# JiapengWu/TeMP

Hardware: AMD Instinct MI355X
Metric: edges/sec (fwd+bwd) RGCN+GRU seq_len=15 (higher is better)
Workload: dtype f32

## Files before the change

### include/temp_amd.h

```cpp
#ifndef TEMP_AMD_H
#define TEMP_AMD_H

#include <stddef.h>
#include <stdint.h>

#ifdef __cplusplus
extern "C" {
#endif

#define TEMP_ABI_VERSION 2

enum {
  TEMP_OK = 0,
  TEMP_E_BADARG = 1,
  TEMP_E_UNSUPPORTED = 2,
  TEMP_E_WORKSPACE = 3,
  TEMP_E_LAUNCH = 4
};

enum { TEMP_ACT_NONE = 0, TEMP_ACT_RELU = 1 };
enum { TEMP_GRU_TORCH = 0,
       TEMP_GRU_TYPE1 = 1 };

int temp_abi_version(void);
// ... 183 lines not shown
size_t temp_gru_bwd_workspace(int n, int d, int variant);
int temp_gru_bwd(int n, int d, int variant,
                 const float* x, const float* prev, const int32_t* prev_idx , const float* dt,
                 float lambda, const float* decay_wb ,
                 const float* w_ih, const float* w_hh,
                 const float* saved, const float* d_h_out,
                 float* d_x, float* d_prev, float* d_w_ih, float* d_w_hh, float* d_b_ih, float* d_b_hh,
                 float* d_decay_wb ,
                 void* workspace, size_t workspace_bytes, void* stream);

int temp_decay_rows(int n, int d, const float* x, const float* dt, float lambda, float* out, void* stream);

int temp_gru_input_gates(int n, int d, int variant, const float* x, const float* w_ih, const float* b_ih, float* gi, void* stream);
int temp_gru_input_gates_multi(int count, const int* ns, int d, int variant, const float* const* xs, const float* const* w_ihs,
                               const float* const* b_ihs, float* const* gis, void* stream);
int temp_gru_input_gates_gather_multi(int count, const int* ns, int d, int variant, const float* const* xs, const int32_t* const* x_idx,
                                      const float* const* w_ihs, const float* const* b_ihs, float* const* gis, void* stream);
int temp_gru_cell_fwd(int n, int d, int variant, const float* gi, const float* prev, const int32_t* prev_idx ,
                      const float* dt, float lambda, const float* w_hh, const float* b_hh,
                      float* h_out, float* saved, size_t saved_plane, void* stream);
int temp_gru_cell_bwd(int n, int d, int variant, const float* saved, size_t saved_plane,
                      const float* dh_up , const float* d_prev_next , const int32_t* next_idx ,
                      const float* dt, float lambda, const float* w_hh,
                      float* dgi, float* dgh, float* decv, float* d_prev, void* stream);
typedef struct TempGruCellFwd {
  int32_t n; const float* gi; const float* prev ;
  const int32_t* prev_idx ; const float* dt;
  const float* w_hh; const float* b_hh; float* h_out; float* saved ;
} TempGruCellFwd;
typedef struct TempGruCellBwd {
  int32_t n; const float* saved; const float* dh_up ; const float* d_prev_next ;
  const int32_t* next_idx ; const float* dt; const float* w_hh;
  float* dgi; float* dgh; float* decv; float* d_prev;
  int32_t no_prev;
} TempGruCellBwd;
int temp_gru_cell_fwd_multi(int count, const TempGruCellFwd* cells, int d, int variant, float lambda, size_t saved_plane, void* stream);
int temp_gru_cell_bwd_multi(int count, const TempGruCellBwd* cells, int d, int variant, float lambda, size_t saved_plane, void* stream);
size_t temp_gru_weight_grads_workspace(int n, int d, int variant);
int temp_gru_weight_grads(int n, int d, int variant, const float* x, const float* hdec, const float* dgi, const float* dgh,
                          const float* w_ih, float* d_x , float* d_w_ih, float* d_w_hh, float* d_b_ih, float* d_b_hh,
                          void* workspace, size_t workspace_bytes, void* stream);
size_t temp_gru_weight_grads_multi_workspace(int count, const int* ns, int d, int variant);
int temp_gru_weight_grads_multi(int count, const int* ns, int d, int variant, const float* const* xs, const float* const* hdecs,
                                const float* const* dgis, const float* const* dghs, const float* const* w_ihs, float* const* d_xs,
                                float* d_w, float* d_b, void* workspace, size_t workspace_bytes, void* stream);

size_t temp_gru_grads_g4_workspace(int count, const int* ns, int d);
int temp_gru_grads_g4(int count, const int* ns, int d, const float* const* xs, const float* const* hdecs, const float* const* g4s,
                      const float* const* w_ihs, float* const* d_xs, float* d_w, float* d_b, void* workspace, size_t workspace_bytes,
                      void* stream);
int temp_gru_grads_g4_keys(int count, const int* ns, int d, const float* const* xs, const float* const* hdecs, const float* const* g4s,
                           const float* const* w_ihs, float* const* d_xs, float* d_w, float* d_b, const uint32_t* const* g4_row_keys,
                           const uint32_t* const* g4_col_keys, const uint32_t* const* x_col_keys ,
                           void* workspace, size_t workspace_bytes, void* stream);
int temp_gru_grads_g4_rows_supported(int count, const int* ns, int d, int table_rows);
int temp_gru_grads_g4_rows(int count, const int* ns, int d, const float* table, int table_rows, const int32_t* const* x_rows,
                           const float* const* hdecs, const float* const* g4s, const float* const* w_ihs, float* const* d_xs, float* d_w,
                           float* d_b, const uint32_t* const* g4_row_keys, const uint32_t* const* g4_col_keys,
                           const uint32_t* const* x_col_keys, void* workspace, size_t workspace_bytes, void* stream);

#define TEMP_CHAIN_HAS_PREV (1 << 30)
#define TEMP_CHAIN_TRACKS 32
#define TEMP_CHAIN_MAX_RNN 4
#define TEMP_CHAIN_MAX_UP 8
typedef struct TempChainDecay { const float* wb[TEMP_CHAIN_MAX_RNN]; } TempChainDecay;
typedef struct TempChainOffset { const float* table; const int32_t* index; int32_t n_rows; } TempChainOffset;
typedef struct TempGruChain {
  int32_t d, variant, n_panels, n_steps;
  int32_t max_steps;
  const int32_t* panel; const int32_t* rows; const int32_t* sinfo;
  const float* dt;
  float lambda;
  size_t saved_plane;
  int32_t n_rnn;
  const float* packed[TEMP_CHAIN_MAX_RNN];
  const float* b_hh[TEMP_CHAIN_MAX_RNN];
  const int32_t* gi_index;
  int32_t pack_layout;
  const TempChainDecay* decay;
  const TempChainOffset* offset;
} TempGruChain;
enum { TEMP_CHAIN_PACK_F32 = 1, TEMP_CHAIN_PACK_BX = 2, TEMP_CHAIN_PACK_HX = 3, TEMP_CHAIN_PACK_HX_X = 4 };
int temp_gru_chain_pack_layout(int d);
int temp_gru_chain_supported(int d);
size_t temp_gru_chain_pack_floats(int d);
int temp_gru_chain_pack(int d, const float* w_hh, float* packed, void* stream);
int temp_gru_chain_pack_multi(int count, int d, const float* const* w_hh, float* const* packed, void* stream);
int temp_gru_chain_pack_multi_layout(int layout, int count, int d, const float* const* w_hh, float* const* packed, void* stream);
size_t temp_gru_chain_pack_x_floats(int d);
int temp_gru_chain_pack_x_multi(int count, int d, const float* const* w_hh, const float* const* w_ih, float* const* packed, void* stream);
typedef struct TempChainFwd {
  const float* gi; const float* x; const int32_t* x_index; const float* const* b_ih;
  float* h_out; float* saved;
} TempChainFwd;
int temp_gru_chain_fwd(const TempGruChain* c, const TempChainFwd* io, void* stream);
typedef struct TempChainBwd {
  const float* saved; int32_t n_up; const float* const* up;
  float* dgi; float* dgh; float* g4; uint32_t* row_keys; uint32_t* col_keys;
  float* d_arg; float* d_state;
} TempChainBwd;
int temp_gru_chain_bwd(const TempGruChain* c, const TempChainBwd* io, void* stream);
int temp_gru_chain_fwd_x_supported(int d, int variant, int max_steps);
long long temp_gru_chain_fwd_x_launches(void);
int temp_gru_chain_keys_supported(int d);
int temp_gru_chain_decay_supported(int d, int variant);
long long temp_gru_chain_decay_launches(void);
int temp_gru_chain_offset_supported(int d, int variant);
int temp_gru_chain_offset_layout(int d);
long long temp_gru_chain_offset_launches(void);
size_t temp_gru_chain_decay_reduce_workspace(const TempGruChain* c);
int temp_gru_chain_decay_reduce(const TempGruChain* c, const float* d_arg, float* d_wb, void* ws, size_t ws_bytes, void* stream);

int temp_gather_rows(int n, int d, const float* table, const int32_t* idx, float* out, void* stream);
size_t temp_keys_cols_size(int d);
int temp_absmax_keys(int n, int d, const float* x, int ldx, uint32_t* row_keys, uint32_t* col_keys, void* stream);
int temp_gather_rows_keys(int n, int d, const float* table, const int32_t* idx, float* out, uint32_t* row_keys, uint32_t* col_keys, void* stream);
int temp_linear_keys(int M, int N, int K, const float* A, int lda, const uint32_t* a_keys, const float* B, int ldb, int trans_b, float* C, int ldc,
                     void* stream);
int temp_gru_input_gates_gather_multi_keys(int count, const int* ns, int d, int variant, const float* const* xs, const int32_t* const* x_idx,
                                           const uint32_t* const* x_keys, const float* const* w_ihs, const float* const* b_ihs, float* const* gis,
                                           void* stream);
int temp_scatter_add_rows(int n, int d, const float* src, const int32_t* idx, float* table, void* stream);
size_t temp_segment_sum_rows_workspace(int n_seg, int n_rows, int d);
int temp_segment_sum_rows(int n_seg, int n_rows, int d, const int32_t* seg_ptr, const int32_t* order, const float* src, float* out,
                          void* workspace, size_t workspace_bytes, void* stream);
int temp_segment_sum_rows_relu(int n_seg, int n_rows, int d, const int32_t* seg_ptr, const int32_t* order, const float* src, const float* relu_of,
                               float* out, void* workspace, size_t workspace_bytes, void* stream);

int temp_diachronic_rows_fwd(int B, int N, int d, const float* ent, const float* w, const float* b, const float* t, float* out, void* stream);
int temp_diachronic_rows_bwd(int B, int N, int d, const float* ent, const float* w, const float* b, const float* t, const float* d_out, float* d_ent,
                             float* d_w, float* d_b, void* stream);

#define TEMP_HYPERPLANE_TILE_ROWS 32
#define TEMP_HYPERPLANE_CHUNK 8
size_t temp_hyperplane_rows_bwd_workspace(int B, int N, int d);
int temp_hyperplane_rows_fwd(int B, int N, int d, const float* table, const float* w, float* out, void* stream);
int temp_hyperplane_rows_bwd(int B, int N, int d, const float* table, const float* w, const float* d_out, float* d_table, float* d_w,
                             void* workspace, size_t workspace_bytes, void* stream);

int temp_linear(int M, int N, int K, const float* A, int lda, const float* B, int ldb, int trans_b, float* C, int ldc, void* stream);
int temp_linear_t(int M, int N, int K, const float* A, int lda, const float* B, int ldb, int trans_b, float* Ct, int ldct, void* stream);
typedef struct TempLinearProblem { int M; const float* A; const float* B; float* C; } TempLinearProblem;
int temp_linear_multi(int count, const TempLinearProblem* probs, int N, int K, int lda, int ldb, int trans_b, int ldc, void* stream);
// ... 124 lines not shown
```

### temp_amd/_lib.py

```python
import ctypes
import threading
import os

_HERE = os.path.dirname(os.path.abspath(__file__))
LIB_PATH = os.path.join(_HERE, "libtemp_amd.so")

c_i32p = ctypes.POINTER(ctypes.c_int32)
c_f32p = ctypes.POINTER(ctypes.c_float)
c_vp = ctypes.c_void_p

ACT_NONE, ACT_RELU = 0, 1
GRU_TORCH, GRU_TYPE1 = 0, 1
CHUNK = 64
CHUNK_REL = 128


class TempEdgeView(ctypes.Structure):
    _fields_ = [("n_seg", ctypes.c_int32), ("n_edges", ctypes.c_int32), ("a", c_vp), ("b", c_vp),
                ("n_chunks", ctypes.c_int32), ("chunk_seg", c_vp), ("chunk_beg", c_vp), ("chunk_end", c_vp),
                ("chunk_slot", c_vp), ("n_partial", ctypes.c_int32), ("n_fix", ctypes.c_int32),
                ("fix_seg", c_vp), ("fix_slot", c_vp), ("fix_cnt", c_vp)]


class TempMembers(ctypes.Structure):
    _fields_ = [("n_members", ctypes.c_int32), ("max_nodes", ctypes.c_int32), ("max_edges", ctypes.c_int32),
                ("max_chunks", ctypes.c_int32 * 3), ("node_off", c_vp), ("edge_off", c_vp), ("chunk_off", c_vp), ("fix_off", c_vp)]


class TempGraph(ctypes.Structure):
    _fields_ = [("n_nodes", ctypes.c_int32), ("n_edges", ctypes.c_int32), ("nnorm", c_vp), ("in_deg", c_vp),
                ("out_deg", c_vp), ("by_dst", TempEdgeView), ("by_src", TempEdgeView), ("by_rel", TempEdgeView),
                ("members", TempMembers)]


class TempPairView(ctypes.Structure):
    _fields_ = [("n_table", ctypes.c_int32), ("n_rel_rows", ctypes.c_int32), ("fwd_row", c_vp), ("by_pair", TempEdgeView)]


ABI_VERSION = 2
OPT_MFMA_BF16X3, OPT_TN_SPLIT, OPT_RGCN_SCALAR, OPT_GEMM_STREAM, OPT_GRU_STREAM, OPT_RGCN_TILE, OPT_DEBUG, OPT_OVERLAP, OPT_GEMM_RESIDENT, OPT_MFMA_F16X2, OPT_RGCN_PAIR = range(11)


class TempGruCellFwd(ctypes.Structure):
    _fields_ = [("n", ctypes.c_int32), ("gi", c_vp), ("prev", c_vp), ("prev_idx", c_vp), ("dt", c_vp), ("w_hh", c_vp),
                ("b_hh", c_vp), ("h_out", c_vp), ("saved", c_vp)]


class TempGruCellBwd(ctypes.Structure):
    _fields_ = [("n", ctypes.c_int32), ("saved", c_vp), ("dh_up", c_vp), ("d_prev_next", c_vp), ("next_idx", c_vp), ("dt", c_vp),
                ("w_hh", c_vp), ("dgi", c_vp), ("dgh", c_vp), ("decv", c_vp), ("d_prev", c_vp), ("no_prev", ctypes.c_int32)]


CHAIN_HAS_PREV = 1 << 30
CHAIN_TRACKS = 32
CHAIN_MAX_RNN = 4
CHAIN_MAX_UP = 8
CHAIN_MAX_STEPS = 64
CHAIN_PACK_F32, CHAIN_PACK_BX, CHAIN_PACK_HX, CHAIN_PACK_HX_X = 1, 2, 3, 4


class TempChainDecay(ctypes.Structure):
    _fields_ = [("wb", c_vp * CHAIN_MAX_RNN)]


class TempChainOffset(ctypes.Structure):
    _fields_ = [("table", c_vp), ("index", c_vp), ("n_rows", ctypes.c_int32)]


class TempGruChain(ctypes.Structure):
    _fields_ = [("d", ctypes.c_int32), ("variant", ctypes.c_int32), ("n_panels", ctypes.c_int32), ("n_steps", ctypes.c_int32),
                ("max_steps", ctypes.c_int32), ("panel", c_vp), ("rows", c_vp), ("sinfo", c_vp), ("dt", c_vp), ("lambda_", ctypes.c_float),
                ("saved_plane", ctypes.c_size_t), ("n_rnn", ctypes.c_int32), ("packed", c_vp * CHAIN_MAX_RNN), ("b_hh", c_vp * CHAIN_MAX_RNN),
                ("gi_index", c_vp), ("pack_layout", ctypes.c_int32),
                ("decay", ctypes.POINTER(TempChainDecay)), ("offset", ctypes.POINTER(TempChainOffset))]


class TempChainFwd(ctypes.Structure):
    _fields_ = [(n, c_vp) for n in ("gi", "x", "x_index", "b_ih", "h_out", "saved")]


class TempChainBwd(ctypes.Structure):
    _fields_ = [("saved", c_vp), ("n_up", ctypes.c_int32), ("up", c_vp)] + [(n, c_vp) for n in ("dgi", "dgh", "g4", "row_keys", "col_keys", "d_arg", "d_state")]


class TempSubsampleJob(ctypes.Structure):
    _fields_ = [("n_nodes", ctypes.c_int32), ("n_edges", ctypes.c_int32), ("keep", ctypes.c_int32), ("seed", ctypes.c_uint64),
                ("parent", c_vp), ("child", c_vp), ("eid", c_vp),
                ("off_a", ctypes.c_int32 * 3), ("off_b", ctypes.c_int32 * 3), ("off_chunk_beg", ctypes.c_int32 * 3),
                ("off_chunk_end", ctypes.c_int32 * 3), ("off_chunk_seg", ctypes.c_int32 * 3), ("n_chunks", ctypes.c_int32 * 3),
                ("off_in_deg", ctypes.c_int32), ("off_out_deg", ctypes.c_int32), ("off_nnorm", ctypes.c_int32),
                ("keep_mask", c_vp), ("scratch", c_vp)]


class TempDropout(ctypes.Structure):
    _fields_ = [("p", ctypes.c_float), ("seed", ctypes.c_uint64)]


class TempAttn(ctypes.Structure):
    _fields_ = [("n", ctypes.c_int32), ("D", ctypes.c_int32), ("heads", ctypes.c_int32), ("T", ctypes.c_int32),
                ("q", c_vp), ("ldq", ctypes.c_int32), ("kh", c_vp), ("vh", c_vp), ("ldh", ctypes.c_int32),
                ("kc", c_vp), ("vc", c_vp), ("ldc", ctypes.c_int32), ("idx", c_vp), ("decay", c_vp)]


class TempAttnSplit(ctypes.Structure):
    _fields_ = [("pa", c_vp), ("ia", c_vp), ("lda", ctypes.c_int32), ("pb", c_vp), ("ib", c_vp), ("ldb", ctypes.c_int32)]


class TempLinearProblem(ctypes.Structure):
    _fields_ = [("M", ctypes.c_int32), ("A", c_vp), ("B", c_vp), ("C", c_vp)]


# ... 18 lines not shown
    "temp_get_option": (_I, [_I]),
    "temp_scratch_refused": (ctypes.c_longlong, []),
    "temp_f16_launches": (ctypes.c_longlong, []),
    "temp_gemm_route_launches": (ctypes.c_longlong, [_I, _I]),
    "temp_rgcn_route_launches": (ctypes.c_longlong, [_I, _I]),
    "temp_tile_launches": (ctypes.c_longlong, []),
    "temp_set_debug_buffer": (None, [c_vp, _SZ]),
    "temp_rgcn_fwd_workspace": (_SZ, [_G, _I]),
    "temp_rgcn_fwd": (_I, [_G, c_vp, c_vp, _I, _I, _I, _I, c_vp, c_vp, c_vp, _I, c_vp, c_vp, _SZ, c_vp, c_vp]),
    "temp_rgcn_bwd_workspace": (_SZ, [_G, _I, _I, _I, _I]),
    "temp_rgcn_bwd": (_I, [_G, c_vp, c_vp, c_vp, _I, _I, _I, _I, c_vp, c_vp, _I, _I, c_vp, c_vp, c_vp, c_vp, c_vp, _SZ, c_vp, c_vp]),
    "temp_rgcn_bwd_dh": (_I, [_G, c_vp, c_vp, _I, _I, _I, _I, c_vp, c_vp, _I, c_vp, c_vp, c_vp, c_vp, _SZ, c_vp, c_vp]),
    "temp_rgcn_bwd_weights": (_I, [_G, c_vp, c_vp, c_vp, _I, _I, _I, _I, _I, c_vp, c_vp, c_vp, c_vp, _SZ, c_vp]),
    "temp_rgcn_table_fwd_workspace": (_SZ, [_G, _I, _I]),
    "temp_rgcn_table_fwd": (_I, [_G, c_vp, c_vp, _I, _I, _I, _I, _I, c_vp, c_vp, c_vp, _I, c_vp, c_vp, _SZ, c_vp, c_vp]),
    "temp_rgcn_table_bwd_workspace": (_SZ, [_G, _I, _I, _I, _I]),
    "temp_rgcn_table_bwd": (_I, [_G, c_vp, c_vp, c_vp, c_vp, _I, c_vp, c_vp, _I, _I, _I, _I, c_vp, c_vp, _I, _I, c_vp, c_vp, c_vp, c_vp,
                                 c_vp, _SZ, c_vp, c_vp]),
    "temp_pair_launches": (ctypes.c_longlong, []),
    "temp_expand_chunk_segments": (_I, [_I, c_vp, c_vp, c_vp, _I, c_vp, c_vp]),
    "temp_rgcn_pair_supported": (_I, [_I, _I, _I]),
    "temp_rgcn_pair_fwd_workspace": (_SZ, [_G, _PV, _I]),
    "temp_rgcn_pair_fwd": (_I, [_G, _PV, c_vp, c_vp, _I, _I, _I, _I, _I, c_vp, c_vp, c_vp, _I, c_vp, c_vp, _SZ, c_vp, c_vp]),
    "temp_rgcn_pair_bwd_workspace": (_SZ, [_G, _PV, _I, _I, _I]),
    "temp_rgcn_pair_bwd": (_I, [_G, _PV, c_vp, c_vp, c_vp, c_vp, _I, c_vp, c_vp, _I, _I, _I, _I, c_vp, c_vp, _I, _I, c_vp, c_vp, c_vp, c_vp,
                                c_vp, _SZ, c_vp, c_vp]),
    "temp_rgcn_isolated_fwd": (_I, [_I, _I, c_vp, c_vp, c_vp, _I, c_vp, c_vp, c_vp]),
    "temp_rgcn_isolated_bwd_workspace": (_SZ, [_I, _I]),
    "temp_rgcn_isolated_bwd": (_I, [_I, _I, c_vp, c_vp, c_vp, c_vp, _I, _I, c_vp, c_vp, c_vp, c_vp, _SZ, c_vp, c_vp]),
    "temp_gru_fwd": (_I, [_I, _I, _I, c_vp, c_vp, c_vp, c_vp, _F, c_vp, c_vp, c_vp, c_vp, c_vp, c_vp, c_vp, c_vp]),
    "temp_gru_bwd_workspace": (_SZ, [_I, _I, _I]),
    "temp_gru_bwd": (_I, [_I, _I, _I, c_vp, c_vp, c_vp, c_vp, _F, c_vp, c_vp, c_vp, c_vp, c_vp,
                          c_vp, c_vp, c_vp, c_vp, c_vp, c_vp, c_vp, c_vp, _SZ, c_vp]),
    "temp_decay_rows": (_I, [_I, _I, c_vp, c_vp, _F, c_vp, c_vp]),
    "temp_gru_input_gates": (_I, [_I, _I, _I, c_vp, c_vp, c_vp, c_vp, c_vp]),
    "temp_gru_input_gates_multi": (_I, [_I, c_vp, _I, _I, c_vp, c_vp, c_vp, c_vp, c_vp]),
    "temp_gru_input_gates_gather_multi": (_I, [_I, c_vp, _I, _I, c_vp, c_vp, c_vp, c_vp, c_vp, c_vp]),
    "temp_gru_cell_fwd": (_I, [_I, _I, _I, c_vp, c_vp, c_vp, c_vp, _F, c_vp, c_vp, c_vp, c_vp, _SZ, c_vp]),
    "temp_gru_cell_bwd": (_I, [_I, _I, _I, c_vp, _SZ, c_vp, c_vp, c_vp, c_vp, _F, c_vp, c_vp, c_vp, c_vp, c_vp, c_vp]),
    "temp_gru_cell_fwd_multi": (_I, [_I, ctypes.POINTER(TempGruCellFwd), _I, _I, _F, _SZ, c_vp]),
    "temp_gru_cell_bwd_multi": (_I, [_I, ctypes.POINTER(TempGruCellBwd), _I, _I, _F, _SZ, c_vp]),
    "temp_gru_weight_grads_workspace": (_SZ, [_I, _I, _I]),
    "temp_gru_weight_grads": (_I, [_I, _I, _I, c_vp, c_vp, c_vp, c_vp, c_vp, c_vp, c_vp, c_vp, c_vp, c_vp, c_vp, _SZ, c_vp]),
    "temp_gru_weight_grads_multi_workspace": (ctypes.c_size_t, [_I, c_vp, _I, _I]),
    "temp_gru_weight_grads_multi": (_I, [_I, c_vp, _I, _I, c_vp, c_vp, c_vp, c_vp, c_vp, c_vp, c_vp, c_vp, c_vp, ctypes.c_size_t, c_vp]),
    "temp_gru_chain_supported": (_I, [_I]),
    "temp_gru_chain_pack_floats": (_SZ, [_I]),
    "temp_gru_chain_pack": (_I, [_I, c_vp, c_vp, c_vp]),
    "temp_gru_chain_pack_multi": (_I, [_I, _I, ctypes.POINTER(c_vp), ctypes.POINTER(c_vp), c_vp]),
    "temp_gru_chain_fwd": (_I, [ctypes.POINTER(TempGruChain), ctypes.POINTER(TempChainFwd), c_vp]),
    "temp_gru_chain_pack_layout": (_I, [_I]),
    "temp_gru_chain_fwd_x_supported": (_I, [_I, _I, _I]),
    "temp_gru_chain_pack_x_floats": (_SZ, [_I]),
    "temp_gru_chain_pack_x_multi": (_I, [_I, _I, ctypes.POINTER(c_vp), ctypes.POINTER(c_vp), ctypes.POINTER(c_vp), c_vp]),
    "temp_gru_chain_fwd_x_launches": (ctypes.c_longlong, []),
    "temp_gru_chain_bwd": (_I, [ctypes.POINTER(TempGruChain), ctypes.POINTER(TempChainBwd), c_vp]),
    "temp_gru_chain_keys_supported": (_I, [_I]),
    "temp_gru_chain_decay_supported": (_I, [_I, _I]),
    "temp_gru_chain_decay_reduce_workspace": (_SZ, [ctypes.POINTER(TempGruChain)]),
    "temp_gru_chain_decay_reduce": (_I, [ctypes.POINTER(TempGruChain), c_vp, c_vp, c_vp, _SZ, c_vp]),
    "temp_gru_chain_decay_launches": (ctypes.c_longlong, []),
    "temp_gru_chain_offset_supported": (_I, [_I, _I]),
    "temp_gru_chain_offset_layout": (_I, [_I]),
    "temp_gru_chain_pack_multi_layout": (_I, [_I, _I, _I, ctypes.POINTER(c_vp), ctypes.POINTER(c_vp), c_vp]),
    "temp_gru_chain_offset_launches": (ctypes.c_longlong, []),
    "temp_gru_grads_g4_keys": (_I, [_I, c_vp, _I, c_vp, c_vp, c_vp, c_vp, c_vp, c_vp, c_vp, c_vp, c_vp, c_vp, c_vp, ctypes.c_size_t, c_vp]),
    "temp_gru_grads_g4_rows_supported": (_I, [_I, c_vp, _I, _I]),
    "temp_gru_grads_g4_rows": (_I, [_I, c_vp, _I, c_vp, _I, c_vp, c_vp, c_vp, c_vp, c_vp, c_vp, c_vp, c_vp, c_vp, c_vp, c_vp, ctypes.c_size_t, c_vp]),
    "temp_gru_grads_g4_workspace": (ctypes.c_size_t, [_I, c_vp, _I]),
    "temp_gru_grads_g4": (_I, [_I, c_vp, _I, c_vp, c_vp, c_vp, c_vp, c_vp, c_vp, c_vp, c_vp, ctypes.c_size_t, c_vp]),
    "temp_gather_rows": (_I, [_I, _I, c_vp, c_vp, c_vp, c_vp]),
    "temp_keys_cols_size": (_SZ, [_I]),
    "temp_absmax_keys": (_I, [_I, _I, c_vp, _I, c_vp, c_vp, c_vp]),
    "temp_gather_rows_keys": (_I, [_I, _I, c_vp, c_vp, c_vp, c_vp, c_vp, c_vp]),
    "temp_linear_keys": (_I, [_I, _I, _I, c_vp, _I, c_vp, c_vp, _I, _I, c_vp, _I, c_vp]),
    "temp_gru_input_gates_gather_multi_keys": (_I, [_I, c_vp, _I, _I, c_vp, c_vp, c_vp, c_vp, c_vp, c_vp, c_vp]),
    "temp_scatter_add_rows": (_I, [_I, _I, c_vp, c_vp, c_vp, c_vp]),
    "temp_segment_sum_rows_workspace": (_SZ, [_I, _I, _I]),
    "temp_segment_sum_rows": (_I, [_I, _I, _I, c_vp, c_vp, c_vp, c_vp, c_vp, _SZ, c_vp]),
    "temp_segment_sum_rows_relu": (_I, [_I, _I, _I, c_vp, c_vp, c_vp, c_vp, c_vp, c_vp, _SZ, c_vp]),
    "temp_diachronic_rows_fwd": (_I, [_I, _I, _I, c_vp, c_vp, c_vp, c_vp, c_vp, c_vp]),
    "temp_diachronic_rows_bwd": (_I, [_I, _I, _I, c_vp, c_vp, c_vp, c_vp, c_vp, c_vp, c_vp, c_vp, c_vp]),
    "temp_hyperplane_rows_bwd_workspace": (_SZ, [_I, _I, _I]),
    "temp_hyperplane_rows_fwd": (_I, [_I, _I, _I, c_vp, c_vp, c_vp, c_vp]),
    "temp_hyperplane_rows_bwd": (_I, [_I, _I, _I, c_vp, c_vp, c_vp, c_vp, c_vp, c_vp, _SZ, c_vp]),
    "temp_linear": (_I, [_I, _I, _I, c_vp, _I, c_vp, _I, _I, c_vp, _I, c_vp]),
    "temp_linear_t": (_I, [_I, _I, _I, c_vp, _I, c_vp, _I, _I, c_vp, _I, c_vp]),
    "temp_linear_multi": (_I, [_I, ctypes.POINTER(TempLinearProblem), _I, _I, _I, _I, _I, _I, c_vp]),
    "temp_linear_tn_workspace": (_SZ, [_I, _I, _I]),
    "temp_linear_tn_multi_workspace": (_SZ, [_I, _I, _I, _I]),
    "temp_linear_tn_multi": (_I, [_I, ctypes.POINTER(TempLinearProblem), _I, _I, _I, _I, _I, c_vp, _SZ, c_vp]),
    "temp_linear_tn": (_I, [_I, _I, _I, c_vp, _I, c_vp, _I, c_vp, _I, c_vp, _SZ, c_vp]),
    "temp_gather_ce_fwd": (_I, [_I, _I, _I, c_vp, c_vp, c_vp, c_vp, c_vp]),
    "temp_gather_ce_bwd": (_I, [_I, _I, _I, c_vp, c_vp, c_vp, c_vp, _F, c_vp, c_vp, c_vp]),
    "temp_bilinear_query_fwd": (_I, [_I, _I, _I, c_vp, c_vp, c_vp, c_vp, c_vp, c_vp, c_vp]),
    "temp_bilinear_query_bwd": (_I, [_I, _I, _I, c_vp, c_vp, c_vp, c_vp, c_vp, c_vp, c_vp, c_vp, c_vp]),
    "temp_l1_ce_fwd": (_I, [_I, _I, _I, c_vp, c_vp, c_vp, c_vp, c_vp, c_vp, c_vp, c_vp]),
    "temp_l1_ce_bwd_q": (_I, [_I, _I, _I, c_vp, c_vp, c_vp, c_vp, c_vp, c_vp, c_vp, _F, c_vp, c_vp, c_vp, c_vp]),
    "temp_l1_ce_bwd_table": (_I, [_I, _I, _I, c_vp, c_vp, c_vp, c_vp, c_vp, c_vp, c_vp]),
    "temp_l1_scores": (_I, [_I, _I, _I, c_vp, c_vp, _I, c_vp, c_vp]),
    "temp_gated_query_fwd": (_I, [_I, _I, _I, c_vp, c_vp, c_vp, c_vp, c_vp, c_vp, c_vp, c_vp, c_vp, c_vp]),
    "temp_gated_query_bwd": (_I, [_I, _I, _I, c_vp, c_vp, c_vp, c_vp, c_vp, c_vp, c_vp, c_vp, c_vp, c_vp, c_vp, c_vp, c_vp, c_vp]),
    "temp_gather_ce_mix_fwd": (_I, [_I, _I, _I, c_vp, c_vp, c_vp, c_vp, c_vp, c_vp, c_vp]),
    "temp_gather_ce_mix_bwd": (_I, [_I, _I, _I, c_vp, c_vp, c_vp, c_vp, c_vp, c_vp, _F, c_vp, c_vp, c_vp, c_vp, c_vp]),
    "temp_l1_mix_ce_fwd": (_I, [_I, _I, _I, c_vp, c_vp, c_vp, c_vp, c_vp, c_vp, c_vp, c_vp, c_vp, c_vp]),
    "temp_l1_mix_ce_bwd_q": (_I, [_I, _I, _I, c_vp, c_vp, c_vp, c_vp, c_vp, c_vp, c_vp, c_vp, c_vp, _F, c_vp, c_vp, c_vp, c_vp, c_vp]),
    "temp_l1_mix_ce_bwd_table": (_I, [_I, _I, _I, c_vp, c_vp, c_vp, c_vp, c_vp, c_vp, c_vp, c_vp, c_vp, c_vp]),
    "temp_l1_mix_scores": (_I, [_I, _I, _I, c_vp, c_vp, c_vp, c_vp, _I, c_vp, c_vp]),
    "temp_assemble_views": (_I, [_I, c_vp, c_vp, c_vp, c_vp, c_vp, c_vp]),
    "temp_subsample_views": (_I, [_I, ctypes.POINTER(TempSubsampleJob), c_vp]),
    "temp_corrupt_sample": (_I, [_I, _I, _I, ctypes.c_uint64, c_vp, c_vp, c_vp, c_vp, c_vp, c_vp]),
    "temp_filtered_rank": (_I, [_I, _I, _I, c_vp, c_vp, c_vp, c_vp, c_vp, c_vp]),
    "temp_filtered_topk": (_I, [_I, _I, _I, _I, _I, c_vp, c_vp, c_vp, c_vp, _I, c_vp, c_vp, c_vp]),
    "temp_filtered_topk_mix": (_I, [_I, _I, _I, _I, _I, c_vp, c_vp, c_vp, c_vp, c_vp, c_vp, _I, c_vp, c_vp, c_vp]),
    "temp_grad_norm_workspace": (_SZ, [_I]),
    "temp_grad_norm_clip": (_I, [_I, _I, c_vp, ctypes.c_double, c_vp, _SZ, c_vp, c_vp]),
    "temp_adam_clip_step": (_I, [_I, _I, c_vp, c_vp, c_vp]),
    "temp_sa_attn_fwd": (_I, [ctypes.POINTER(TempAttn), c_vp, c_vp, c_vp, c_vp]),
    "temp_sa_attn_bwd": (_I, [ctypes.POINTER(TempAttn), c_vp, c_vp, c_vp, c_vp, c_vp, _I, c_vp, c_vp, _I, c_vp, c_vp, _I, c_vp, _I, c_vp, c_vp, c_vp, c_vp]),
    "temp_sa_attn_split_fwd": (_I, [ctypes.POINTER(TempAttn), ctypes.POINTER(TempAttnSplit), c_vp, c_vp, c_vp, c_vp]),
    "temp_sa_attn_split_bwd": (_I, [ctypes.POINTER(TempAttn), ctypes.POINTER(TempAttnSplit), c_vp, c_vp, c_vp, c_vp, c_vp, _I, c_vp, c_vp, _I, c_vp,
# ... 151 lines not shown
```

### temp_amd/backend.py

```python
import ctypes

import torch

from . import _lib

_backend = None


def set_backend(b):
    global _backend
    _backend = b


def get_backend():
    global _backend
    if _backend is None:
        _backend = HipBackend()
    return _backend


def _ptr(t):
    return ctypes.c_void_p(t.data_ptr()) if t is not None else None


# ... 414 lines not shown
            decay = _f32(decay, "decay")
            assert decay.numel() == 2
            cd = _lib.TempChainDecay()
            for i in range(c.n_rnn):
                cd.wb[i] = decay.data_ptr()
            c.decay = ctypes.pointer(cd)
            keep += [cd, decay]
        if offset is not None:
            table, index = _f32(offset[0], "offset table"), _i32(offset[1], "offset index")
            assert table.dim() == 2 and table.shape[1] == d and index.numel() * d == plane
            co = _lib.TempChainOffset()
            co.table, co.index, co.n_rows = table.data_ptr(), index.data_ptr(), table.shape[0]
            c.offset = ctypes.pointer(co)
            keep += [co, table, index]
        return c, keep

    def gru_chain_decay_supported(self, d, variant):
        return bool(self.lib.temp_gru_chain_decay_supported(int(d), int(variant)))

    def gru_chain_decay_launches(self):
        return int(self.lib.temp_gru_chain_decay_launches())

    def gru_chain_decay_reduce(self, tabs, d, variant, d_arg, n_rnn):
        c, keep = self._chain_desc(tabs, d, variant, n_rnn=n_rnn)
        d_arg = _f32(d_arg, "d_arg")
        out = torch.empty(n_rnn, 2, dtype=torch.float32, device=d_arg.device)
        nb = int(self.lib.temp_gru_chain_decay_reduce_workspace(ctypes.byref(c)))
        ws = torch.empty(max(nb, 4) // 4, dtype=torch.float32, device=d_arg.device)
        _lib.check(self.lib.temp_gru_chain_decay_reduce(ctypes.byref(c), _ptr(d_arg), _ptr(out), _ptr(ws), nb, _stream()), "temp_gru_chain_decay_reduce")
        return out

    def gru_chain_offset_supported(self, d, variant):
        return bool(self.lib.temp_gru_chain_offset_supported(int(d), int(variant)))

    def gru_chain_offset_layout(self, d):
        return int(self.lib.temp_gru_chain_offset_layout(int(d)))

    def gru_chain_offset_launches(self):
        return int(self.lib.temp_gru_chain_offset_launches())

    def gru_chain_fwd(self, tabs, gi, lam, variant, packs, b_hhs, h_out, saved_all, gi_index=None, decay=None, offset=None):
        d = saved_all.shape[2]
        c, keep = self._chain_desc(tabs, d, variant, lam, saved_all.shape[1] * d, packs, b_hhs, decay, offset)
        if gi_index is not None:
            assert gi_index.shape[0] == saved_all.shape[1]
            c.gi_index = _i32(gi_index, "gi_index").data_ptr()
        gi = _f32(gi, "gi")
        io = _lib.TempChainFwd(gi=gi.data_ptr(), h_out=h_out.data_ptr(), saved=saved_all.data_ptr())
        _lib.check(self.lib.temp_gru_chain_fwd(ctypes.byref(c), ctypes.byref(io), _stream()), "temp_gru_chain_fwd")

    def gru_chain_fwd_x_supported(self, d, variant, max_steps):
        return bool(self.lib.temp_gru_chain_fwd_x_supported(int(d), int(variant), int(max_steps)))

    def gru_chain_pack_x_multi(self, w_hhs, w_ihs):
        w_hhs, w_ihs = [_f32(w, "w_hh") for w in w_hhs], [_f32(w, "w_ih") for w in w_ihs]
        d = w_hhs[0].shape[1]
        k = len(w_hhs)
        n = self.lib.temp_gru_chain_pack_x_floats(d)
        buf = torch.empty(k, n, dtype=torch.float32, device=w_hhs[0].device)
        arr = lambda ts: (ctypes.c_void_p * k)(*[t.data_ptr() for t in ts])
        _lib.check(self.lib.temp_gru_chain_pack_x_multi(k, d, arr(w_hhs), arr(w_ihs), arr([buf[i] for i in range(k)]), _stream()),
                   "temp_gru_chain_pack_x_multi")
        return self._tagged([buf[i] for i in range(k)], _lib.CHAIN_PACK_HX_X)

    def gru_chain_fwd_x(self, tabs, x, x_index, lam, variant, packs, b_hhs, b_ihs, h_out, saved_all, decay=None):
        d = saved_all.shape[2]
        c, keep = self._chain_desc(tabs, d, variant, lam, saved_all.shape[1] * d, packs, b_hhs, decay)
        x, x_index = _f32(x, "x"), _i32(x_index, "x_index")
        assert x.shape[1] == d and x_index.shape[0] == saved_all.shape[1]
        b_ihs = [_f32(b, "b_ih") for b in b_ihs]
        barr = (ctypes.c_void_p * len(b_ihs))(*[b.data_ptr() for b in b_ihs])
        io = _lib.TempChainFwd(x=x.data_ptr(), x_index=x_index.data_ptr(), b_ih=ctypes.addressof(barr), h_out=h_out.data_ptr(), saved=saved_all.data_ptr())
        _lib.check(self.lib.temp_gru_chain_fwd(ctypes.byref(c), ctypes.byref(io), _stream()), "temp_gru_chain_fwd (x route)")

    def _chain_bwd(self, tabs, saved_all, ups, lam, variant, packs, b_hhs, decay, d_arg, offset, d_state, **out):
        d = saved_all.shape[2]
        c, keep = self._chain_desc(tabs, d, variant, lam, saved_all.shape[1] * d, packs, b_hhs, decay, offset)
        ups = [_f32(u, "upstream") if u is not None else None for u in ups]
        arr = (ctypes.c_void_p * max(len(ups), 1))(*[u.data_ptr() if u is not None else None for u in ups])
        d_arg = _f32(d_arg, "d_arg")
        if d_state is not None:
            assert d_state.dtype == torch.float32 and d_state.is_contiguous() and d_state.shape == saved_all.shape[1:]
        io = _lib.TempChainBwd(saved=saved_all.data_ptr(), n_up=len(ups), up=ctypes.addressof(arr))
        for name, t in dict(out, d_arg=d_arg, d_state=d_state).items():
            setattr(io, name, t.data_ptr() if t is not None else None)
        _lib.check(self.lib.temp_gru_chain_bwd(ctypes.byref(c), ctypes.byref(io), _stream()), "temp_gru_chain_bwd")

    def gru_chain_bwd(self, tabs, saved_all, ups, lam, variant, packs, b_hhs, dgi, dgh, decay=None, d_arg=None, offset=None, d_state=None):
        self._chain_bwd(tabs, saved_all, ups, lam, variant, packs, b_hhs, decay, d_arg, offset, d_state, dgi=dgi, dgh=dgh)

    def gru_chain_keys_supported(self, d):
        return bool(self.lib.temp_gru_chain_keys_supported(int(d)))

    def gru_chain_bwd_g4(self, tabs, saved_all, ups, lam, variant, packs, b_hhs, g4, keys=None, decay=None, d_arg=None, offset=None, d_state=None):
        row_keys, col_keys = keys if keys is not None else (None, None)
        if keys is not None:
            assert offset is None, "an offset chain hands out no keys (its states are not bounded by the f16 split's constant scale)"
            assert row_keys.dtype == torch.int32 and col_keys.dtype == torch.int32 and col_keys.is_contiguous()
            assert row_keys.numel() == saved_all.shape[1] and col_keys.numel() == (len(packs) + tabs["n_panels"]) * 4 * saved_all.shape[2]
        self._chain_bwd(tabs, saved_all, ups, lam, variant, packs, b_hhs, decay, d_arg, offset, d_state, g4=g4, row_keys=row_keys, col_keys=col_keys)

    def gru_grads_g4_supported(self, ns, d, variant):
        k = len(ns)
        if k < 1 or k > 4 or variant != _lib.GRU_TORCH:
            return False
        return self.lib.temp_gru_grads_g4_workspace(k, (ctypes.c_int * k)(*[int(n) for n in ns]), int(d)) > 0

    def gru_grads_g4(self, xs, hdecs, g4s, w_ihs, d_xs, row_keys=None, col_keys=None, x_col_keys=None):
        k = len(xs)
        d = xs[0].shape[1]
        dev = xs[0].device
        ns = (ctypes.c_int * k)(*[x.shape[0] for x in xs])
        nb = self.lib.temp_gru_grads_g4_workspace(k, ns, d)
        if nb == 0:
            raise ValueError("temp_gru_grads_g4: unsupported shape (check gru_grads_g4_supported first)")
        keep = [[_f32(t, "operand") for t in ts] for ts in (xs, hdecs, w_ihs)]
        for g in g4s:
            assert g.dtype == torch.float32 and g.is_contiguous() and g.shape[1] == 4 * d
        arr = lambda ts: (ctypes.c_void_p * k)(*[t.data_ptr() for t in ts])
        dx = (ctypes.c_void_p * k)(*[None if t is None else t.data_ptr() for t in d_xs])
        d_w = torch.empty(2 * k, 3 * d, d, dtype=torch.float32, device=dev)
        d_b = torch.empty(2 * k, 3 * d, dtype=torch.float32, device=dev)
        ws = self._ws(nb, dev)
        if row_keys is not None and col_keys is not None:
            for rk, ck, x in zip(row_keys, col_keys, xs):
                assert rk.dtype == torch.int32 and ck.dtype == torch.int32 and rk.is_contiguous() and ck.is_contiguous()
                assert rk.numel() == x.shape[0] and ck.numel() == 4 * d
            xk = None
            if x_col_keys is not None:
                for t in x_col_keys:
                    assert t.dtype == torch.int32 and t.is_contiguous() and t.numel() == d
                xk = arr(x_col_keys)
            rc = self.lib.temp_gru_grads_g4_keys(k, ns, d, arr(keep[0]), arr(keep[1]), arr(g4s), arr(keep[2]), dx, _ptr(d_w), _ptr(d_b),
                                                 arr(row_keys), arr(col_keys), xk, _ptr(ws), ws.numel(), _stream())
            _lib.check(rc, "temp_gru_grads_g4_keys")
            return [(d_w[2 * i], d_w[2 * i + 1], d_b[2 * i], d_b[2 * i + 1]) for i in range(k)]
        rc = self.lib.temp_gru_grads_g4(k, ns, d, arr(keep[0]), arr(keep[1]), arr(g4s), arr(keep[2]), dx, _ptr(d_w), _ptr(d_b), _ptr(ws),
                                        ws.numel(), _stream())
        _lib.check(rc, "temp_gru_grads_g4")
        return [(d_w[2 * i], d_w[2 * i + 1], d_b[2 * i], d_b[2 * i + 1]) for i in range(k)]

    def gru_grads_g4_rows_supported(self, ns, d, variant, table_rows):
        k = len(ns)
        if k < 1 or k > 4 or variant != _lib.GRU_TORCH:
            return False
        return bool(self.lib.temp_gru_grads_g4_rows_supported(k, (ctypes.c_int * k)(*[int(n) for n in ns]), int(d), int(table_rows)))

    def gru_grads_g4_rows(self, table, x_rows, hdecs, g4s, w_ihs, d_xs, row_keys, col_keys, x_col_keys):
        table = _f32(table, "table")
        k, d, dev = len(x_rows), table.shape[1], table.device
        ns = (ctypes.c_int * k)(*[r.shape[0] for r in x_rows])
        nb = self.lib.temp_gru_grads_g4_workspace(k, ns, d)
        if nb == 0:
            raise ValueError("temp_gru_grads_g4_rows: unsupported shape (check gru_grads_g4_supported first)")
        x_rows = [_i32(r, "x_rows") for r in x_rows]
        keep = [[_f32(t, "operand") for t in ts] for ts in (hdecs, w_ihs)]
        for g, r, h, rk, ck, xk in zip(g4s, x_rows, keep[0], row_keys, col_keys, x_col_keys):
            assert g.dtype == torch.float32 and g.is_contiguous() and g.shape == (r.shape[0], 4 * d) and h.shape == (r.shape[0], d)
            assert all(t.dtype == torch.int32 and t.is_contiguous() for t in (rk, ck, xk))
            assert rk.numel() == r.shape[0] and ck.numel() == 4 * d and xk.numel() == d
        arr = lambda ts: (ctypes.c_void_p * k)(*[t.data_ptr() for t in ts])
        dx = (ctypes.c_void_p * k)(*[None if t is None else t.data_ptr() for t in d_xs])
        d_w = torch.empty(2 * k, 3 * d, d, dtype=torch.float32, device=dev)
        d_b = torch.empty(2 * k, 3 * d, dtype=torch.float32, device=dev)
        ws = self._ws(nb, dev)
        rc = self.lib.temp_gru_grads_g4_rows(k, ns, d, _ptr(table), table.shape[0], arr(x_rows), arr(keep[0]), arr(g4s), arr(keep[1]), dx,
                                             _ptr(d_w), _ptr(d_b), arr(row_keys), arr(col_keys), arr(x_col_keys), _ptr(ws), ws.numel(), _stream())
        _lib.check(rc, "temp_gru_grads_g4_rows")
        return [(d_w[2 * i], d_w[2 * i + 1], d_b[2 * i], d_b[2 * i + 1]) for i in range(k)]

    def gru_weight_grads(self, x, hdec, dgi, dgh, w_ih, variant, d_x):
        n, d = x.shape
        w_ih = _f32(w_ih, "w_ih")
        dev = x.device
        d_w_ih = torch.empty_like(w_ih)
        d_w_hh = torch.empty(3 * d, d, dtype=torch.float32, device=dev)
        d_b_ih = torch.empty(w_ih.shape[0], dtype=torch.float32, device=dev)
        d_b_hh = torch.empty(3 * d, dtype=torch.float32, device=dev)
        ws = self._ws(self.lib.temp_gru_weight_grads_workspace(n, d, variant), dev)
        rc = self.lib.temp_gru_weight_grads(n, d, variant, _ptr(x), _ptr(hdec), _ptr(dgi), _ptr(dgh), _ptr(w_ih), _ptr(d_x),
                                            _ptr(d_w_ih), _ptr(d_w_hh), _ptr(d_b_ih), _ptr(d_b_hh), _ptr(ws), ws.numel(), _stream())
        _lib.check(rc, "temp_gru_weight_grads")
        return d_w_ih, d_w_hh, d_b_ih, d_b_hh

    def gru_weight_grads_multi(self, xs, hdecs, dgis, dghs, w_ihs, variant, d_xs):
        k = len(xs)
        if k < 1 or k > 4 or variant != _lib.GRU_TORCH or any(h is None for h in hdecs):
            return None
        d = xs[0].shape[1]
        dev = xs[0].device
        ns = (ctypes.c_int * k)(*[x.shape[0] for x in xs])
        nb = self.lib.temp_gru_weight_grads_multi_workspace(k, ns, d, variant)
        if nb == 0:
            return None
        keep = [[_f32(t, "operand") for t in ts] for ts in (xs, hdecs, dgis, dghs, w_ihs)]
        arr = lambda ts: (ctypes.c_void_p * k)(*[t.data_ptr() for t in ts])
        dx = (ctypes.c_void_p * k)(*[None if t is None else t.data_ptr() for t in d_xs])
        d_w = torch.empty(2 * k, 3 * d, d, dtype=torch.float32, device=dev)
        d_b = torch.empty(2 * k, 3 * d, dtype=torch.float32, device=dev)
        ws = self._ws(nb, dev)
        rc = self.lib.temp_gru_weight_grads_multi(k, ns, d, variant, arr(keep[0]), arr(keep[1]), arr(keep[2]), arr(keep[3]), arr(keep[4]), dx,
                                                  _ptr(d_w), _ptr(d_b), _ptr(ws), ws.numel(), _stream())
        if rc == 2:
            return None
        _lib.check(rc, "temp_gru_weight_grads_multi")
        return [(d_w[2 * i], d_w[2 * i + 1], d_b[2 * i], d_b[2 * i + 1]) for i in range(k)]

    def linear(self, a, b, trans_b, out=None, a_keys=None):
        a, b = _f32(a, "a"), _f32(b, "b")
        M, K = a.shape
        N = b.shape[0] if trans_b else b.shape[1]
        c = out if out is not None else torch.empty(M, N, dtype=torch.float32, device=a.device)
        assert c.shape == (M, N) and c.is_contiguous() and c.dtype == torch.float32
        if a_keys is not None:
            assert a_keys.dtype == torch.int32 and a_keys.is_contiguous() and a_keys.numel() == M
            rc = self.lib.temp_linear_keys(M, N, K, _ptr(a), K, _ptr(a_keys), _ptr(b), b.shape[1], int(trans_b), _ptr(c), N, _stream())
            _lib.check(rc, "temp_linear_keys")
            return c
        rc = self.lib.temp_linear(M, N, K, _ptr(a), K, _ptr(b), b.shape[1], int(trans_b), _ptr(c), N, _stream())
        _lib.check(rc, "temp_linear")
# ... 523 lines not shown
```

### temp_amd/csrc/gemm_bx.hpp

```cpp
#pragma once
#include "gemm_panel.hpp"

namespace temp {

typedef __bf16 bx_bf16x8 __attribute__((ext_vector_type(8)));
typedef unsigned int bx_u32x4 __attribute__((ext_vector_type(4)));

__device__ __forceinline__ void bx_split(float x, unsigned& h, unsigned& m, unsigned& l) {
  h = __float_as_uint(x) & 0xffff0000u;
  const float r1 = x - __uint_as_float(h);
  m = __float_as_uint(r1) & 0xffff0000u;
  l = __float_as_uint(r1 - __uint_as_float(m));
}
__device__ __forceinline__ void bx_split2(float x0, float x1, unsigned& H, unsigned& M, unsigned& L) {
  unsigned h0, m0, l0, h1, m1, l1;
  bx_split(x0, h0, m0, l0);
  bx_split(x1, h1, m1, l1);
  H = __builtin_amdgcn_perm(h1, h0, 0x07060302u);
  M = __builtin_amdgcn_perm(m1, m0, 0x07060302u);
  L = __builtin_amdgcn_perm(l1, l0, 0x07060302u);
}
__device__ __forceinline__ void bx_split8(const float4 a, const float4 b, bx_u32x4& H, bx_u32x4& M, bx_u32x4& L) {
  unsigned h, m, l;
  bx_split2(a.x, a.y, h, m, l); H[0] = h; M[0] = m; L[0] = l;
// ... 528 lines not shown
  }
  bx_u32x4* slot = pbytes * n_distinct <= BX_PACK_MAX_BYTES ? bx_scratch(st, pbytes * n_distinct) : nullptr;
  if (!slot) return false;
  const int n_slabs = ceil_div(g.K, 16);
  int done = 0;
  BxPackJobs jobs = {};
  for (int i = 0; i < PANEL_MAXP; ++i) pk->b[i] = slot;
  for (int i = 0; i < count; ++i) {
    bx_u32x4* dst = slot + (size_t)which[i] * (pbytes / 16);
    pk->b[i] = dst;
    if (which[i] < done) continue;
    ++done;
    if (n_distinct > 1 && n_distinct <= BX_PACK_JOBS) { bx_pack_jobs_add(jobs, batch.p[i].B, dst, g.K, g.N, g.ldb, g.trans_b); continue; }
    const dim3 pgrid(ceil_div((long long)n_slabs * g.n_tiles, 4));
    if (g.trans_b) TEMP_LAUNCH(K_BX_PACK, (k_bx_pack<1>), pgrid, dim3(256), 0, st, g.K, g.N, g.n_tiles, n_slabs, batch.p[i].B, g.ldb, dst);
    else TEMP_LAUNCH(K_BX_PACK, (k_bx_pack<0>), pgrid, dim3(256), 0, st, g.K, g.N, g.n_tiles, n_slabs, batch.p[i].B, g.ldb, dst);
  }
  if (jobs.count) TEMP_LAUNCH(K_BX_PACK, k_bx_pack_multi, dim3(ceil_div(jobs.total_units, 4)), dim3(256), 0, st, jobs);
  return true;
}

template <int G, class Epi>
static inline void launch_bx_g(int kid, const PanelBatch<Epi>& batch, int count, const BxGeom& g, hipStream_t st, const BxPacked* pk) {
  dim3 grid(8 * g.per_xcd * g.n_groups, count);
  gemm_route_count(pk ? TEMP_ROUTE_BXP : (g.trans_b ? TEMP_ROUTE_BX_T : TEMP_ROUTE_BX), G);
  if (pk) {
    TEMP_LAUNCH(kid, (k_gemm_bxp<G, Epi>), grid, dim3(BX_THREADS), 0, st, batch, g, *pk);
    return;
  }
  if (g.trans_b) TEMP_LAUNCH(kid, (k_gemm_bx<G, 1, Epi>), grid, dim3(BX_THREADS), 0, st, batch, g);
  else TEMP_LAUNCH(kid, (k_gemm_bx<G, 0, Epi>), grid, dim3(BX_THREADS), 0, st, batch, g);
}

template <class Epi>
static inline bool launch_bxr(int kid, const PanelBatch<Epi>& batch, int count, const BxGeom& g, hipStream_t st, const BxPacked* pkp) {
  if (!option(TEMP_OPT_GEMM_RESIDENT) || g.K > BXR_MAX_SLABS * 16 || g.K < 72) return false;
  if (EpiRawPre<Epi>::value && !EpiAccInit<Epi>::value && !(option(TEMP_OPT_DEBUG) & 0x200000)) return false;
  int max_m = 0;
  for (int i = 0; i < count; ++i) max_m = batch.p[i].M > max_m ? batch.p[i].M : max_m;
  BxrGeom rg;
  if (!bxr_plan(g.N, g.K, g.lda, max_m, &rg)) return false;
  rg.ldb = g.ldb; rg.trans_b = g.trans_b;
  BxPacked pk;
  for (int i = 0; i < PANEL_MAXP; ++i) pk.b[i] = pkp ? pkp->b[i] : nullptr;
  static const bool granted = hipFuncSetAttribute(reinterpret_cast<const void*>(k_gemm_bxr<Epi>), hipFuncAttributeMaxDynamicSharedMemorySize, BXR_LDS_BYTES) == hipSuccess;
  if (!granted) { (void)hipGetLastError(); return false; }
  const size_t lds = (size_t)rg.n_slabs * BXR_G * 192 * 16 + BXR_BIAS_BYTES;
  gemm_route_count(TEMP_ROUTE_BXR, 0);
  TEMP_LAUNCH(kid, (k_gemm_bxr<Epi>), dim3(256, count), dim3(BXR_WAVES * 64), lds, st, batch, rg, pk);
  return true;
}

template <class Epi>
int launch_gemm_bx(int kid, const PanelBatch<Epi>& batch, int count, const BxGeom& g, int G, hipStream_t st) {
  if (launch_hxr(kid, batch, count, g, st)) return launch_status();
  if (launch_bxr(kid, batch, count, g, st, nullptr)) return launch_status();
  if (hx_supported(batch, count, g)) {
    const int rc = launch_gemm_hx(kid, batch, count, g, G, st);
    if (rc != TEMP_E_UNSUPPORTED) return rc;
  }
  BxPacked pk;
  const bool packed = bx_pack_batch(batch, count, g, st, &pk);
  const BxPacked* pp = packed ? &pk : nullptr;
  switch (G) {
    case 1: launch_bx_g<1, Epi>(kid, batch, count, g, st, pp); break;
    case 2: launch_bx_g<2, Epi>(kid, batch, count, g, st, pp); break;
    case 3: launch_bx_g<3, Epi>(kid, batch, count, g, st, pp); break;
    case 4: launch_bx_g<4, Epi>(kid, batch, count, g, st, pp); break;
    case 5: launch_bx_g<5, Epi>(kid, batch, count, g, st, pp); break;
    case 6: launch_bx_g<6, Epi>(kid, batch, count, g, st, pp); break;
    default: launch_bx_g<7, Epi>(kid, batch, count, g, st, pp); break;
  }
  return launch_status();
}

}
```

### temp_amd/csrc/gemm_hx.hpp

```cpp
#pragma once
#include "gemm_bx.hpp"
#include "hx_pack.hpp"

namespace temp {

struct HxPacked { const hx_u32x4* b[PANEL_MAXP]; const unsigned* keys[PANEL_MAXP]; };

template <int G, class Epi>
__global__ void __launch_bounds__(BX_THREADS, (G <= 4 ? 3 : 2)) k_gemm_hxp(PanelBatch<Epi> batch, BxGeom g, HxPacked packed, int keys_by_out) {
  constexpr int PIECES = G * 128;
  constexpr int NPC = (PIECES + BX_THREADS - 1) / BX_THREADS;
  __shared__ __attribute__((aligned(16))) hx_u32x4 Bs[2][PIECES];
  const PanelProblem<Epi>& pb = batch.p[blockIdx.y];
  const int M = pb.M;
  const int xcd = blockIdx.x & 7, local = blockIdx.x >> 3;
  const int grp = local % g.n_groups, rt_local = local / g.n_groups;
  const int rt = xcd * g.per_xcd + rt_local;
  if (rt_local >= g.per_xcd || rt * 128 >= M) return;
  const bool tail = grp == g.n_groups - 1;
  const int t0 = tail ? g.n_tiles - G : grp * G;
  const int t_store = tail ? G - g.tail_store : 0;
  const int n0 = t0 * 32;
  const int N = g.N, K = g.K;
  const float* __restrict__ A = pb.A;
// ... 213 lines not shown
  if (!hx_enabled() || g.K % 4 || g.lda % 4) return false;
  size_t need_keys = 0;
  for (int i = 0; i < count; ++i)
    if (!batch.p[i].a_keys) need_keys += align_up((size_t)(batch.p[i].M > 0 ? batch.p[i].M : 0) * 4, 256);
  if (need_keys > 0 && ceil_div(g.N, 32) < 16 && g.K < 400 && !(option(TEMP_OPT_DEBUG) & 0x800)) return false;
  return need_keys <= BX_SLOT_BYTES - HX_KEYS_OFFSET;
}

template <class Epi>
static inline bool hx_fill_keys(PanelBatch<Epi>& batch, int count, int K, int lda, unsigned char* slot, hipStream_t st, int* keys_by_out) {
  bool any_own = false, any_given_gather = false;
  for (int i = 0; i < count; ++i) {
    if (batch.p[i].M <= 0) continue;
    if (!batch.p[i].a_keys) any_own = true;
    else if (batch.p[i].a_idx) any_given_gather = true;
  }
  if (any_own && any_given_gather) return false;
  size_t koff = HX_KEYS_OFFSET;
  AbsRowsBatch ab = {};
  int n_own = 0, max_own = 0, last = -1;
  for (int i = 0; i < count; ++i) {
    if (batch.p[i].M <= 0) { batch.p[i].a_keys = reinterpret_cast<const unsigned*>(slot + HX_KEYS_OFFSET); continue; }
    if (batch.p[i].a_keys) continue;
    unsigned* keys = reinterpret_cast<unsigned*>(slot + koff);
    koff += align_up((size_t)batch.p[i].M * 4, 256);
    ab.M[n_own] = batch.p[i].M; ab.A[n_own] = batch.p[i].A; ab.idx[n_own] = batch.p[i].a_idx; ab.keys[n_own] = keys;
    max_own = batch.p[i].M > max_own ? batch.p[i].M : max_own;
    ++n_own;
    last = i;
    batch.p[i].a_keys = keys;
  }
  if (n_own == 1) {
    int blocks = ceil_div(batch.p[last].M, 16);
    if (blocks > 2048) blocks = 2048;
    TEMP_LAUNCH(K_KEYS, k_absmax_rows_idx, dim3(blocks), dim3(256), 0, st, ab.M[0], K, ab.A[0], lda, ab.idx[0], ab.keys[0]);
  } else if (n_own > 1) {
    int blocks = ceil_div(max_own, 16);
    if (blocks > 2048 / n_own) blocks = 2048 / n_own;
    TEMP_LAUNCH(K_KEYS, k_absmax_rows_idx_multi, dim3(blocks, n_own), dim3(256), 0, st, ab, K, lda);
  }
  for (int i = count; i < PANEL_MAXP; ++i) batch.p[i].a_keys = batch.p[0].a_keys;
  *keys_by_out = any_own ? 1 : 0;
  return true;
}

template <int G, class Epi>
static inline void launch_hxp_g(int kid, const PanelBatch<Epi>& batch, int count, const BxGeom& g, hipStream_t st, const HxPacked& pk, int keys_by_out) {
  dim3 grid(8 * g.per_xcd * g.n_groups, count);
  gemm_route_count(TEMP_ROUTE_HXP, G);
  TEMP_LAUNCH(kid, (k_gemm_hxp<G, Epi>), grid, dim3(BX_THREADS), 0, st, batch, g, pk, keys_by_out);
}

template <class Epi>
int launch_gemm_hx(int kid, const PanelBatch<Epi>& batch_in, int count, const BxGeom& g, int G, hipStream_t st) {
  const size_t pbytes = align_up(hx_pack_bytes(g.N, g.K), 256);
  int n_distinct = 0, which[PANEL_MAXP];
  for (int i = 0; i < count; ++i) {
    which[i] = -1;
    for (int j = 0; j < i; ++j)
      if (batch_in.p[j].B == batch_in.p[i].B) { which[i] = which[j]; break; }
    if (which[i] < 0) which[i] = n_distinct++;
  }
  if (pbytes * n_distinct > BX_PACK_MAX_BYTES || n_distinct > HX_PACK_JOBS) return TEMP_E_UNSUPPORTED;
  unsigned char* slot = reinterpret_cast<unsigned char*>(bx_scratch(st, BX_SLOT_BYTES));
  if (!slot) return TEMP_E_UNSUPPORTED;
  PanelBatch<Epi> batch = batch_in;
  HxPacked pk;
  HxPackJobs jobs = {};
  const size_t items = hx_packed_items(g.N, g.K);
  int done = 0;
  for (int i = 0; i < PANEL_MAXP; ++i) { pk.b[i] = reinterpret_cast<const hx_u32x4*>(slot); pk.keys[i] = reinterpret_cast<const unsigned*>(slot + items * 16); }
  for (int i = 0; i < count; ++i) {
    unsigned char* dst = slot + (size_t)which[i] * pbytes;
    pk.b[i] = reinterpret_cast<const hx_u32x4*>(dst);
    pk.keys[i] = reinterpret_cast<const unsigned*>(dst + items * 16);
    if (which[i] < done) continue;
    ++done;
    hx_pack_jobs_add(jobs, batch.p[i].B, reinterpret_cast<hx_u32x4*>(dst), reinterpret_cast<unsigned*>(dst + items * 16), g.K, g.N, g.ldb, g.trans_b);
  }
  int kbo = 0;
  if (!hx_fill_keys(batch, count, g.K, g.lda, slot, st, &kbo)) return TEMP_E_UNSUPPORTED;
  hx_pack_launch(jobs, K_BX_PACK, st);
  hx_count();
  switch (G) {
    case 1: launch_hxp_g<1, Epi>(kid, batch, count, g, st, pk, kbo); break;
    case 2: launch_hxp_g<2, Epi>(kid, batch, count, g, st, pk, kbo); break;
    case 3: launch_hxp_g<3, Epi>(kid, batch, count, g, st, pk, kbo); break;
    case 4: launch_hxp_g<4, Epi>(kid, batch, count, g, st, pk, kbo); break;
    case 5: launch_hxp_g<5, Epi>(kid, batch, count, g, st, pk, kbo); break;
    case 6: launch_hxp_g<6, Epi>(kid, batch, count, g, st, pk, kbo); break;
    default: launch_hxp_g<7, Epi>(kid, batch, count, g, st, pk, kbo); break;
  }
  return launch_status();
}

}
#include "gemm_hxr.hpp"
namespace temp {

template <class Epi>
static inline bool launch_hxr(int kid, const PanelBatch<Epi>& batch_in, int count, const BxGeom& g, hipStream_t st) {
  if (!option(TEMP_OPT_GEMM_RESIDENT) || g.K > BXR_MAX_SLABS * 16 || g.K < 72 || g.K % 8 || !hx_supported(batch_in, count, g)) return false;
  int max_m = 0;
  for (int i = 0; i < count; ++i) max_m = batch_in.p[i].M > max_m ? batch_in.p[i].M : max_m;
  BxrGeom rg;
  if (!bxr_plan(g.N, g.K, g.lda, max_m, &rg)) return false;
  rg.ldb = g.ldb; rg.trans_b = g.trans_b;
  static const bool granted = hipFuncSetAttribute(reinterpret_cast<const void*>(k_gemm_hxr<Epi>), hipFuncAttributeMaxDynamicSharedMemorySize, HXR_LDS_BYTES) == hipSuccess;
  if (!granted) { (void)hipGetLastError(); return false; }
  PanelBatch<Epi> batch = batch_in;
  bool need = false;
  for (int i = 0; i < count; ++i) need = need || (batch.p[i].M > 0 && !batch.p[i].a_keys);
  int kbo = 0;
  if (need) {
    unsigned char* slot = reinterpret_cast<unsigned char*>(bx_scratch(st, BX_SLOT_BYTES));
    if (!slot || !hx_fill_keys(batch, count, g.K, g.lda, slot, st, &kbo)) return false;
  } else {
    for (int i = 0; i < PANEL_MAXP; ++i) if (!batch.p[i].a_keys) batch.p[i].a_keys = batch.p[0].a_keys;
    for (int i = 0; i < count; ++i) if (batch.p[i].M > 0) { for (int j = 0; j < PANEL_MAXP; ++j) if (!batch.p[j].a_keys) batch.p[j].a_keys = batch.p[i].a_keys; break; }
  }
  const size_t lds = (size_t)rg.n_slabs * BXR_G * 128 * 16 + 3 * BXR_BIAS_BYTES;
  gemm_route_count(TEMP_ROUTE_HXR, 0);
  TEMP_LAUNCH(kid, (k_gemm_hxr<Epi>), dim3(256, count), dim3(BXR_WAVES * 64), lds, st, batch, rg, kbo);
  hx_count();
  return true;
}

}
```

### temp_amd/csrc/gemm_wres.hpp

```cpp
#pragma once
#include <stdlib.h>
#include <type_traits>
#include "gemm_panel.hpp"
#include "gemm_bx.hpp"

namespace temp {

#define WRES_TPS 3
#define WRES_LDS_BYTES (80 * 1024)
#define WRES_LOCAL_BLOCKS 64

#define WRES_MIN_ROWS 4096
#define WRES_QC 5

struct WresGeom {
  int N, K, lda, ldb, trans_b;
  int ldk;
  int kpad;
  int n_tiles, tps;
  int n_slices;
  int tail_store;
  int gate_stride;
  int split;
};
// ... 215 lines not shown
      bool okA = false, okB = false;
      int kcA = 0, kcB = 0;
      long srcA = -1, srcB = -1;
      setup_ld();
      zero_acc();
      issue(bufA, okA, kcA, srcA);
      while (true) {
        stage(bufA, okA, kcA, srcA, bufB, okB, kcB, srcB);
        if (panel >= p_end) break;
        stage(bufB, okB, kcB, srcB, bufA, okA, kcA, srcA);
        if (panel >= p_end) break;
      }
    }
    if constexpr (VAR & 8) epi.stamp(4, __builtin_amdgcn_s_memtime());
  }
}

template <int NTS, class Epi>
int launch_wres_one(int kid, const PanelBatch<Epi>& batch, int count, const WresGeom& g, hipStream_t st, int local_blocks = WRES_LOCAL_BLOCKS) {
  static bool attr_set = false;
  if (!attr_set) {
    if (hipFuncSetAttribute((const void*)k_gemm_wres<NTS, Epi>, hipFuncAttributeMaxDynamicSharedMemorySize, WRES_LDS_BYTES) != hipSuccess)
      return TEMP_E_LAUNCH;
    attr_set = true;
  }
  const int roles = g.n_slices * (g.split ? count : 1);
  const size_t lds = (size_t)NTS * 32 * g.ldk * 4;
  if (local_blocks == WRES_LOCAL_BLOCKS) {
    int per_cu = (int)((160 * 1024) / (lds + 1024));
    if (per_cu > 3) per_cu = 3;
    if (per_cu > 2) local_blocks = 32 * per_cu;
  }
  int bps = local_blocks / roles;
  if (bps < 1) bps = 1;
  int max_m = 0;
  for (int i = 0; i < count; ++i) max_m = batch.p[i].M > max_m ? batch.p[i].M : max_m;
  const int need = ceil_div(ceil_div(ceil_div(max_m, 32), 8), 4);
  if (bps > need) bps = need < 1 ? 1 : need;
  gemm_route_count(g.split ? TEMP_ROUTE_WRES_SPLIT : TEMP_ROUTE_WRES, NTS);
  TEMP_LAUNCH(kid, (k_gemm_wres<NTS, Epi>), dim3(roles * bps * 8), dim3(256), lds, st, batch, count, g, bps);
  return launch_status();
}

template <class Epi>
int launch_gemm_wres(int kid, const PanelBatch<Epi>& batch, int count, const WresGeom& g, hipStream_t st) {
  if (g.tps == 3) return launch_wres_one<3, Epi>(kid, batch, count, g, st);
  if (g.tps == 2) return launch_wres_one<2, Epi>(kid, batch, count, g, st);
  return launch_wres_one<1, Epi>(kid, batch, count, g, st);
}

inline bool wres_disabled() { return option(TEMP_OPT_GEMM_STREAM) != 0; }

template <class Epi>
int launch_gemm_panel_multi(int kid, const PanelBatch<Epi>& batch, int count, int N, int K, int lda, int ldb, int trans_b, hipStream_t st) {
  if (count <= 0 || count > PANEL_MAXP) return TEMP_E_BADARG;
  long long rows = 0;
  for (int i = 0; i < count; ++i) rows += batch.p[i].M > 0 ? batch.p[i].M : 0;
  if (rows <= 0 || N <= 0) return TEMP_OK;
  if constexpr (!EpiIsGroup<Epi>::value) {
    if (bx_enabled()) {
      int max_m = 0;
      for (int i = 0; i < count; ++i) max_m = batch.p[i].M > max_m ? batch.p[i].M : max_m;
      BxGeom bg;
      int G;
      if (bx_plan(N, K, lda, ldb, trans_b, max_m, rows, &bg, &G)) return launch_gemm_bx(kid, batch, count, bg, G, st);
      if (K % 8 == 4 && bx_plan(N, K, lda, ldb, trans_b, max_m, rows, &bg, &G, true) && hx_supported(batch, count, bg)) {
        const int rc = launch_gemm_hx(kid, batch, count, bg, G, st);
        if (rc != TEMP_E_UNSUPPORTED) return rc;
      }
    }
  }
  WresGeom g;
  if (!wres_disabled() && wres_plan(N, K, lda, ldb, trans_b, rows, &g)) {
    bool distinct = count > 1;
    for (int i = 1; i < count; ++i) distinct = distinct && batch.p[i].B != batch.p[i - 1].B;
    if (distinct && g.n_slices * count <= WRES_LOCAL_BLOCKS) g.split = 1;
    return launch_gemm_wres(kid, batch, count, g, st);
  }
  return launch_gemm_stream_multi(kid, batch, count, N, K, lda, ldb, trans_b, st);
}

template <class Epi>
int launch_gemm_panel(int kid, int M, int N, int K, const float* A, int lda, const int32_t* a_idx, const float* B, int ldb, int trans_b,
                      const Epi& epi, hipStream_t st) {
  if (M <= 0 || N <= 0) return TEMP_OK;
  PanelBatch<Epi> batch;
  for (int i = 0; i < PANEL_MAXP; ++i) batch.p[i] = PanelProblem<Epi>{0, nullptr, nullptr, nullptr, epi};
  batch.p[0] = PanelProblem<Epi>{M, A, a_idx, B, epi};
  return launch_gemm_panel_multi(kid, batch, 1, N, K, lda, ldb, trans_b, st);
}

}
```

### temp_amd/csrc/gru_chain.hip

```cpp
#include <atomic>
#include "common.hpp"
#include "gru_math.hpp"
#include "gemm_bx.hpp"

namespace temp {

#define CH_SLOTS TEMP_CHAIN_TRACKS
#define CH_HAS_PREV TEMP_CHAIN_HAS_PREV
#define CH_ROW_MASK (TEMP_CHAIN_HAS_PREV - 1)
#define CH_LDS_LIMIT (160 * 1024)

struct ChainRnn {
  const float4* wf; const float4* wb; const float* b_hh; const unsigned* kf; const unsigned* kb;
  const float* decay_wb;
};
struct ChainArgs {
  int D, n_panels, max_steps, dbg;
  int layout;
  int n_rnn_keys;
  const int32_t* panel; const int32_t* rows; const int32_t* sinfo;
  const float* dt;
  const int32_t* gi_index;
  float lambda;
  size_t plane;
// ... 615 lines not shown
    if (e >= 0 && (e & CH_HAS_PREV)) {
      const int row = e & CH_ROW_MASK;
      const float g = d_arg[row];
      dw = fmaf(g, dt[row], dw);
      db += g;
    }
  }
  red[threadIdx.x] = make_float2(dw, db);
  __syncthreads();
  for (int w = CH_DECAY_THREADS / 2; w > 0; w >>= 1) {
    if ((int)threadIdx.x < w) { red[threadIdx.x].x += red[threadIdx.x + w].x; red[threadIdx.x].y += red[threadIdx.x + w].y; }
    __syncthreads();
  }
  if (threadIdx.x == 0) part[p] = red[0];
}
__global__ void __launch_bounds__(64) k_chain_decay_final(int n_panels, const int32_t* __restrict__ panel, const float2* __restrict__ part, float2* __restrict__ d_wb) {
  __shared__ float2 red[64];
  const int r = blockIdx.x;
  float dw = 0.f, db = 0.f;
  for (int p = threadIdx.x; p < n_panels; p += 64)
    if (panel[4 * p] == r) { dw += part[p].x; db += part[p].y; }
  red[threadIdx.x] = make_float2(dw, db);
  __syncthreads();
  for (int w = 32; w > 0; w >>= 1) {
    if ((int)threadIdx.x < w) { red[threadIdx.x].x += red[threadIdx.x + w].x; red[threadIdx.x].y += red[threadIdx.x + w].y; }
    __syncthreads();
  }
  if (threadIdx.x == 0) d_wb[r] = red[0];
}

static bool chain_layout_ok(int layout, int d);
static int chain_check(const TempGruChain* c) {
  if (!c || c->d <= 0 || c->n_panels < 0 || c->n_steps < 0 || c->n_rnn <= 0 || c->n_rnn > TEMP_CHAIN_MAX_RNN) return TEMP_E_BADARG;
  if (c->variant != TEMP_GRU_TORCH && c->variant != TEMP_GRU_TYPE1) return TEMP_E_BADARG;
  if (c->n_panels > 0 && (!c->panel || !c->rows || !c->sinfo || !c->dt)) return TEMP_E_BADARG;
  for (int i = 0; i < c->n_rnn; ++i) if (!c->packed[i] || !c->b_hh[i]) return TEMP_E_BADARG;
  if (c->max_steps <= 0 || c->max_steps > CH_MAX_STEPS) return TEMP_E_BADARG;
  if (!temp_gru_chain_supported(c->d)) return TEMP_E_UNSUPPORTED;
  if (!chain_layout_ok(c->pack_layout, c->d)) return TEMP_E_BADARG;
  return TEMP_OK;
}

static bool chain_bx(int d) { return bx_enabled() && d % 8 == 0; }
static bool chain_hx_fits(int d) {
  if (d % 8) return false;
  const ChainGeomHx g = chain_geom_hx(d);
  return chain_lds_fwd_hx(d, CH_MAX_STEPS) <= CH_LDS_LIMIT && chain_lds_bwd_hx(d, CH_MAX_STEPS) <= CH_LDS_LIMIT && g.NT <= 20 && g.NTb <= 8;
}
static bool chain_hx(int d) { return chain_bx(d) && hx_enabled() && chain_hx_fits(d); }
static int chain_pack_layout(int d) { return chain_hx(d) ? TEMP_CHAIN_PACK_HX : chain_bx(d) ? TEMP_CHAIN_PACK_BX : TEMP_CHAIN_PACK_F32; }
static bool chain_layout_ok(int layout, int d) {
  if (layout == TEMP_CHAIN_PACK_F32) return true;
  if (layout == TEMP_CHAIN_PACK_BX) return d % 8 == 0;
  return (layout == TEMP_CHAIN_PACK_HX || layout == TEMP_CHAIN_PACK_HX_X) && chain_hx_fits(d);
}
static bool layout_hx(int layout) { return layout == TEMP_CHAIN_PACK_HX || layout == TEMP_CHAIN_PACK_HX_X; }

static ChainArgs chain_args(const TempGruChain* c, float* d_arg = nullptr, float* d_state = nullptr) {
  ChainArgs a = {};
  a.d_arg = d_arg;
  if (c->offset) { a.off_table = c->offset->table; a.off_index = c->offset->index; a.off_rows = c->offset->n_rows; }
  a.d_state = d_state;
  const ChainGeom g = chain_geom(c->d);
  a.D = c->d; a.n_panels = c->n_panels; a.max_steps = c->max_steps; a.panel = c->panel; a.rows = c->rows; a.sinfo = c->sinfo; a.dt = c->dt;
  a.layout = c->pack_layout;
  a.n_rnn_keys = c->n_rnn; a.lambda = c->lambda; a.plane = c->saved_plane; a.gi_index = c->gi_index; a.dbg = option(TEMP_OPT_DEBUG) >> 8; a.stamp = debug_buffer_chain(CHX_STAMP_WORDS);
  for (int i = 0; i < c->n_rnn; ++i) {
    a.rnn[i].wf = (const float4*)c->packed[i];
    a.rnn[i].wb = (const float4*)c->packed[i] + (a.layout == TEMP_CHAIN_PACK_BX ? (size_t)(g.NQ >> 1) * g.NT * 192 : (size_t)g.NT * g.NQ * 64);
    a.rnn[i].b_hh = c->b_hh[i];
    a.rnn[i].decay_wb = c->decay ? c->decay->wb[i] : nullptr;
    a.rnn[i].kf = a.rnn[i].kb = nullptr;
    if (layout_hx(a.layout)) {
      const ChainGeomHx gx = chain_geom_hx(c->d);
      a.rnn[i].wb = (const float4*)c->packed[i] + chain_hx_fwd_items(c->d);
      a.rnn[i].kf = (const unsigned*)((const float4*)c->packed[i] + chain_hx_fwd_items(c->d) + chain_hx_bwd_items(c->d));
      a.rnn[i].kb = a.rnn[i].kf + gx.NT * 32;
    }
  }
  return a;
}

template <class K>
static int chain_lds_attr(K kernel, size_t bytes, bool* done) {
  if (*done) return TEMP_OK;
  if (hipFuncSetAttribute((const void*)kernel, hipFuncAttributeMaxDynamicSharedMemorySize, CH_LDS_LIMIT) != hipSuccess) return TEMP_E_LAUNCH;
  (void)bytes;
  *done = true;
  return TEMP_OK;
}

template <int VARIANT, int TPW>
static int launch_chain_fwd(const ChainArgs& a, const float* gi, float* h, float* saved, hipStream_t st) {
  static bool attr = false;
  static bool attr_bx = false;
  static bool attr_hx = false;
  if (layout_hx(a.layout)) {
    const size_t lds_hx = chain_lds_fwd_hx(a.D, a.max_steps);
    constexpr int TPW8 = (TPW * 4 + 7) / 8 < 1 ? 1 : (TPW * 4 + 7) / 8;
    const int cfg = (a.dbg >> 4) & 3;
    if (cfg == 1) {
      auto kernel = k_gru_chain_fwd_hx<VARIANT, TPW, 4, 4>;
      int rc = chain_lds_attr(kernel, lds_hx, &attr_hx);
      if (rc) return rc;
      TEMP_LAUNCH(K_GRU_CHAIN_FWD, kernel, dim3(a.n_panels), dim3(512), lds_hx, st, a, gi, h, saved);
    } else if (cfg == 2) {
      static bool attr_48 = false;
      auto kernel = k_gru_chain_fwd_hx<VARIANT, TPW, 8, 4>;
      int rc = chain_lds_attr(kernel, lds_hx, &attr_48);
// ... 197 lines not shown
  }
  TEMP_LAUNCH(K_GRU_CHAIN_PACK, k_bx_pack_multi, dim3(ceil_div(jobs.total_units, 4)), dim3(256), 0, (hipStream_t)stream, jobs);
  return launch_status();
}

}

static std::atomic<long long> g_decay_launches{0};
static std::atomic<long long> g_offset_launches{0};
static void chain_count(const TempGruChain* c) {
  if (c->decay) g_decay_launches.fetch_add(1, std::memory_order_relaxed);
  if (c->offset) g_offset_launches.fetch_add(1, std::memory_order_relaxed);
}
static int chain_decay_check(const TempGruChain* c) {
  if (!c->decay) return TEMP_OK;
  for (int i = 0; i < c->n_rnn; ++i) if (!c->decay->wb[i]) return TEMP_E_BADARG;
  return temp_gru_chain_decay_supported(c->d, c->variant) ? TEMP_OK : TEMP_E_UNSUPPORTED;
}
static int chain_offset_check(const TempGruChain* c) {
  if (!c->offset) return TEMP_OK;
  if (!c->offset->table || !c->offset->index || c->offset->n_rows <= 0) return TEMP_E_BADARG;
  if (!temp_gru_chain_offset_supported(c->d, c->variant)) return TEMP_E_UNSUPPORTED;
  return layout_hx(c->pack_layout) ? TEMP_E_UNSUPPORTED : TEMP_OK;
}
static int chain_desc_check(const TempGruChain* c, const void* io) {
  int rc = io ? chain_check(c) : TEMP_E_BADARG;
  if (!rc) rc = chain_decay_check(c);
  if (!rc) rc = chain_offset_check(c);
  return rc;
}

static int chain_fwd_gi(const TempGruChain* c, const TempChainFwd* io, hipStream_t st) {
  if (c->n_panels == 0) return TEMP_OK;
  if (!io->gi || !io->h_out || !io->saved) return TEMP_E_BADARG;
  const ChainArgs a = chain_args(c);
  chain_count(c);
  const int tpw = ceil_div(chain_geom(c->d).NT, 4);
#define TEMP_CHAIN_FWD(V)                                                            \
  switch (tpw) {                                                                     \
    case 1: return launch_chain_fwd<V, 1>(a, io->gi, io->h_out, io->saved, st);      \
    case 2: return launch_chain_fwd<V, 2>(a, io->gi, io->h_out, io->saved, st);      \
    case 3: return launch_chain_fwd<V, 3>(a, io->gi, io->h_out, io->saved, st);      \
    case 4: return launch_chain_fwd<V, 4>(a, io->gi, io->h_out, io->saved, st);      \
    case 5: return launch_chain_fwd<V, 5>(a, io->gi, io->h_out, io->saved, st);      \
    case 6: return launch_chain_fwd<V, 6>(a, io->gi, io->h_out, io->saved, st);      \
    default: return TEMP_E_UNSUPPORTED;                                              \
  }
  if (c->variant == TEMP_GRU_TORCH) { TEMP_CHAIN_FWD(TEMP_GRU_TORCH) }
  TEMP_CHAIN_FWD(TEMP_GRU_TYPE1)
#undef TEMP_CHAIN_FWD
}

static int chain_fwd_x(const TempGruChain* c, const TempChainFwd* io, hipStream_t st) {
  if (c->pack_layout != TEMP_CHAIN_PACK_HX_X) return TEMP_E_BADARG;
  if (c->variant != TEMP_GRU_TORCH || !chain_fwd_x_fits(c->d, c->max_steps)) return TEMP_E_UNSUPPORTED;
  if (c->n_panels == 0) return TEMP_OK;
  if (!io->x_index || !io->b_ih || !io->h_out || !io->saved) return TEMP_E_BADARG;
  for (int i = 0; i < c->n_rnn; ++i) if (!io->b_ih[i]) return TEMP_E_BADARG;
  const ChainArgs a = chain_args(c);
  chain_count(c);
  int rc = TEMP_OK;
  ChainX X = {};
  X.x = io->x; X.x_index = io->x_index;
  const ChainGeomHx gx = chain_geom_hx(c->d);
  for (int i = 0; i < c->n_rnn; ++i) {
    X.b_ih[i] = io->b_ih[i];
    X.wi[i] = reinterpret_cast<const hx_u32x4*>(c->packed[i] + chain_x_ih_offset(c->d));
  }
  const size_t lds = chain_lds_fwd_x(c->d, c->max_steps);
  const bool dev = a.stamp || (a.dbg & (1 | 2 | 4 | 64 | 2048 | 4096));
  const int tpw = (gx.NT + 7) / 8;
  auto launch = [&](auto kernel, bool* granted) {
    if ((rc = chain_lds_attr(kernel, lds, granted))) return rc;
    TEMP_LAUNCH(K_GRU_CHAIN_FWD, kernel, dim3(a.n_panels), dim3(1024), lds, st, a, X, io->h_out, io->saved);
    return (int)TEMP_OK;
  };
  static bool attr3 = false, attr2 = false, attr1 = false, attr3d = false, attr2d = false, attr1d = false;
  if (tpw == 3) rc = dev ? launch(k_gru_chain_fwd_x<3, 8, 8, 1>, &attr3d) : launch(k_gru_chain_fwd_x<3, 8, 8>, &attr3);
  else if (tpw == 2) rc = dev ? launch(k_gru_chain_fwd_x<2, 8, 8, 1>, &attr2d) : launch(k_gru_chain_fwd_x<2, 8, 8>, &attr2);
  else rc = dev ? launch(k_gru_chain_fwd_x<1, 8, 8, 1>, &attr1d) : launch(k_gru_chain_fwd_x<1, 8, 8>, &attr1);
  if (rc) return rc;
  hx_count();
  g_fwd_x_launches.fetch_add(1, std::memory_order_relaxed);
  return launch_status();
}

static int chain_bwd(const TempGruChain* c, const TempChainBwd* io, hipStream_t st) {
  const bool keys = io->row_keys || io->col_keys;
  if (io->d_state && !c->offset) return TEMP_E_BADARG;
  if (io->n_up < 0 || io->n_up > TEMP_CHAIN_MAX_UP || (io->n_up > 0 && !io->up)) return TEMP_E_BADARG;
  if ((c->decay != nullptr) != (io->d_arg != nullptr)) return TEMP_E_BADARG;
  if (io->g4 ? (io->dgi || io->dgh) : keys) return TEMP_E_BADARG;
  if (io->g4 && c->variant != TEMP_GRU_TORCH) return TEMP_E_UNSUPPORTED;
  if (keys && !layout_hx(c->pack_layout)) return TEMP_E_UNSUPPORTED;
  if (c->n_panels == 0) return TEMP_OK;
  if (!io->saved || (!io->g4 && (!io->dgi || !io->dgh))) return TEMP_E_BADARG;
  const ChainArgs a = chain_args(c, io->d_arg, io->d_state);
  chain_count(c);
  ChainUps ups = {};
  for (int i = 0; i < io->n_up; ++i) ups.p[i] = io->up[i];
  const int tpw = ceil_div(chain_geom(c->d).NTb, 4);
  if (io->g4) {
    if (tpw == 1) return launch_chain_bwd<TEMP_GRU_TORCH, 1, 1>(a, ups, io->saved, io->g4, nullptr, st, io->row_keys, io->col_keys);
    if (tpw == 2) return launch_chain_bwd<TEMP_GRU_TORCH, 2, 1>(a, ups, io->saved, io->g4, nullptr, st, io->row_keys, io->col_keys);
    return TEMP_E_UNSUPPORTED;
  }
  if (c->variant == TEMP_GRU_TORCH) {
    if (tpw == 1) return launch_chain_bwd<TEMP_GRU_TORCH, 1>(a, ups, io->saved, io->dgi, io->dgh, st);
    if (tpw == 2) return launch_chain_bwd<TEMP_GRU_TORCH, 2>(a, ups, io->saved, io->dgi, io->dgh, st);
  } else {
    if (tpw == 1) return launch_chain_bwd<TEMP_GRU_TYPE1, 1>(a, ups, io->saved, io->dgi, io->dgh, st);
    if (tpw == 2) return launch_chain_bwd<TEMP_GRU_TYPE1, 2>(a, ups, io->saved, io->dgi, io->dgh, st);
  }
  return TEMP_E_UNSUPPORTED;
}

extern "C" {

int temp_gru_chain_fwd(const TempGruChain* c, const TempChainFwd* io, void* stream) {
  const int rc = chain_desc_check(c, io);
  if (rc) return rc;
  if (io->gi && io->x) return TEMP_E_BADARG;
  return io->x ? chain_fwd_x(c, io, (hipStream_t)stream) : chain_fwd_gi(c, io, (hipStream_t)stream);
}
int temp_gru_chain_bwd(const TempGruChain* c, const TempChainBwd* io, void* stream) {
  const int rc = chain_desc_check(c, io);
  return rc ? rc : chain_bwd(c, io, (hipStream_t)stream);
}

int temp_gru_chain_offset_supported(int d, int variant) {
  return (variant == TEMP_GRU_TORCH || variant == TEMP_GRU_TYPE1) && temp_gru_chain_supported(d) ? 1 : 0;
}
int temp_gru_chain_offset_layout(int d) { return d > 0 ? (chain_bx(d) ? TEMP_CHAIN_PACK_BX : TEMP_CHAIN_PACK_F32) : 0; }
long long temp_gru_chain_offset_launches(void) { return g_offset_launches.load(std::memory_order_relaxed); }
int temp_gru_chain_decay_supported(int d, int variant) {
  return (variant == TEMP_GRU_TORCH || variant == TEMP_GRU_TYPE1) && temp_gru_chain_supported(d) ? 1 : 0;
}
long long temp_gru_chain_decay_launches(void) { return g_decay_launches.load(std::memory_order_relaxed); }
long long temp_gru_chain_fwd_x_launches(void) { return g_fwd_x_launches.load(std::memory_order_relaxed); }
int temp_gru_chain_pack_layout(int d) { return d > 0 ? chain_pack_layout(d) : 0; }
int temp_gru_chain_keys_supported(int d) { return d > 0 && chain_hx(d) ? 1 : 0; }

int temp_gru_chain_fwd_x_supported(int d, int variant, int max_steps) {
  return d > 0 && d % 8 == 0 && variant == TEMP_GRU_TORCH && chain_fwd_x_ok(d, max_steps) ? 1 : 0;
}

size_t temp_gru_chain_pack_x_floats(int d) {
  if (d <= 0) return 0;
  return chain_x_ih_offset(d) + chain_hx_fwd_items(d) * 4;
}

int temp_gru_chain_pack_x_multi(int count, int d, const float* const* w_hh, const float* const* w_ih, float* const* packed, void* stream) {
  if (count <= 0 || count > TEMP_CHAIN_MAX_RNN || d <= 0 || !w_hh || !w_ih || !packed) return TEMP_E_BADARG;
  for (int i = 0; i < count; ++i) if (!w_hh[i] || !w_ih[i] || !packed[i]) return TEMP_E_BADARG;
  if (d % 8 || !chain_hx(d)) return TEMP_E_UNSUPPORTED;
  const ChainGeomHx gx = chain_geom_hx(d);
  HxPackJobs jobs = {};
  for (int i = 0; i < count; ++i) {
    hx_u32x4* pf = reinterpret_cast<hx_u32x4*>(packed[i]);
    hx_u32x4* pb = pf + chain_hx_fwd_items(d);
    unsigned* kf = reinterpret_cast<unsigned*>(pb + chain_hx_bwd_items(d));
    hx_u32x4* pi = reinterpret_cast<hx_u32x4*>(packed[i] + chain_x_ih_offset(d));
    if (jobs.count + 2 > HX_PACK_JOBS) { hx_pack_launch(jobs, K_GRU_CHAIN_PACK, (hipStream_t)stream); jobs = HxPackJobs{}; }
    hx_pack_jobs_add_joint(jobs, w_hh[i], pf, w_ih[i], pi, kf, d, 3 * d, d, 1);
    hx_pack_jobs_add(jobs, w_hh[i], pb, kf + gx.NT * 32, 3 * d, d, d, 0, gx.NSb);
  }
  hx_pack_launch(jobs, K_GRU_CHAIN_PACK, (hipStream_t)stream);
  return launch_status();
}

size_t temp_gru_chain_decay_reduce_workspace(const TempGruChain* c) {
  if (!c || c->n_panels <= 0) return 0;
  return (size_t)c->n_panels * sizeof(float2);
}

int temp_gru_chain_decay_reduce(const TempGruChain* c, const float* d_arg, float* d_wb, void* ws, size_t ws_bytes, void* stream) {
  if (!c || c->n_panels < 0 || c->n_rnn <= 0 || c->n_rnn > TEMP_CHAIN_MAX_RNN || !d_wb) return TEMP_E_BADARG;
  hipStream_t st = (hipStream_t)stream;
  if (c->n_panels == 0) return hipMemsetAsync(d_wb, 0, (size_t)c->n_rnn * 2 * sizeof(float), st) == hipSuccess ? TEMP_OK : TEMP_E_LAUNCH;
  if (!c->panel || !c->rows || !c->dt || !d_arg) return TEMP_E_BADARG;
  if (!ws || ws_bytes < temp_gru_chain_decay_reduce_workspace(c)) return TEMP_E_WORKSPACE;
  TEMP_LAUNCH(K_GRU_CHAIN_PACK, k_chain_decay_reduce, dim3(c->n_panels), dim3(CH_DECAY_THREADS), 0, st, c->n_panels, c->panel, c->rows, c->dt, d_arg, (float2*)ws);
  TEMP_LAUNCH(K_GRU_CHAIN_PACK, k_chain_decay_final, dim3(c->n_rnn), dim3(64), 0, st, c->n_panels, c->panel, (const float2*)ws, (float2*)d_wb);
  return launch_status();
}

}
```

### temp_amd/csrc/gru_kernels.hip

```cpp
#include "common.hpp"
#include <stdlib.h>
#include "gemm_wres.hpp"
#include "gru_math.hpp"
#include "gru_wgrad_hx.hpp"
#include "side_stream.hpp"

namespace temp {

#define GRU_KC 40
#define GRU_LDB 33

#define GRU_NVB ((3 * GRU_KC * 32 / 4 + 255) / 256)
#define GRU_NQ (GRU_KC / 8)

struct GruPhase {
  const float* W; int row_base[3]; int D; int j0;
};

__device__ __forceinline__ bool gru_w_piece(int i, const GruPhase& ph, int k0, size_t* off) {
  const int p = threadIdx.x + i * 256;
  const int g = p / (32 * GRU_KC / 4), rem = p - g * (32 * GRU_KC / 4);
  const int j = rem / (GRU_KC / 4), k = (rem - j * (GRU_KC / 4)) * 4;
  const int rb = (g == 0) ? ph.row_base[0] : (g == 1 ? ph.row_base[1] : ph.row_base[2]);
  *off = (size_t)(rb + ph.j0 + j) * ph.D + k0 + k;
// ... 795 lines not shown
                          colsum_workspace(n, 3 * d), (hipStream_t)stream);
}

size_t temp_gru_weight_grads_multi_workspace(int count, const int* ns, int d, int variant) {
  if (count <= 0 || count > 4 || !ns || d <= 0 || variant != TEMP_GRU_TORCH) return 0;
  int max_n = 0;
  for (int i = 0; i < count; ++i) {
    if (ns[i] <= 0) return 0;
    max_n = ns[i] > max_n ? ns[i] : max_n;
  }
  if (d % 4 || !gemm_tn_multi_bias_supported(2 * count, max_n, 3 * d, d, 3 * d, d)) return 0;
  return gemm_tn_multi_bias_workspace(2 * count, max_n, 3 * d, d);
}

int temp_gru_weight_grads_multi(int count, const int* ns, int d, int variant, const float* const* xs, const float* const* hdecs,
                                const float* const* dgis, const float* const* dghs, const float* const* w_ihs, float* const* d_xs,
                                float* d_w, float* d_b, void* workspace, size_t workspace_bytes, void* stream) {
  if (count <= 0 || count > 4 || !ns || !xs || !hdecs || !dgis || !dghs || !w_ihs || !d_xs || !d_w || !d_b) return TEMP_E_BADARG;
  if (variant != TEMP_GRU_TORCH || d % 4) return TEMP_E_UNSUPPORTED;
  int max_n = 0;
  for (int i = 0; i < count; ++i) {
    if (ns[i] <= 0 || !xs[i] || !hdecs[i] || !dgis[i] || !dghs[i] || !w_ihs[i]) return TEMP_E_UNSUPPORTED;
    max_n = ns[i] > max_n ? ns[i] : max_n;
  }
  hipStream_t st = (hipStream_t)stream;
  int Ms[8];
  const float* As[8];
  const float* Bs[8];
  for (int i = 0; i < count; ++i) {
    Ms[2 * i] = Ms[2 * i + 1] = ns[i];
    As[2 * i] = dgis[i]; Bs[2 * i] = xs[i];
    As[2 * i + 1] = dghs[i]; Bs[2 * i + 1] = hdecs[i];
  }
  int rc = gemm_tn_multi_bias(2 * count, Ms, 3 * d, d, As, 3 * d, Bs, d, d_w, d_b, workspace, workspace_bytes, st);
  if (rc) return rc;
  PanelBatch<EpiStore> batch;
  int nx = 0;
  for (int i = 0; i < count; ++i)
    if (d_xs[i]) batch.p[nx++] = PanelProblem<EpiStore>{ns[i], dgis[i], nullptr, w_ihs[i], EpiStore{d_xs[i], d}};
  for (int i = nx; i < PANEL_MAXP && nx > 0; ++i) { batch.p[i] = batch.p[0]; batch.p[i].M = 0; }
  if (nx > 0) rc = launch_gemm_panel_multi(K_GEMM_GRU_DX, batch, nx, d, 3 * d, 3 * d, d, 0, st);
  return rc ? rc : launch_status();
}

size_t temp_gru_grads_g4_workspace(int count, const int* ns, int d) {
  WgArgs a = {};
  if (!grads_g4_plan(count, ns, d, &a)) return 0;
  return wg_workspace(a).total;
}

int temp_gru_grads_g4(int count, const int* ns, int d, const float* const* xs, const float* const* hdecs, const float* const* g4s,
                      const float* const* w_ihs, float* const* d_xs, float* d_w, float* d_b, void* workspace, size_t workspace_bytes,
                      void* stream) {
  return temp_gru_grads_g4_keys(count, ns, d, xs, hdecs, g4s, w_ihs, d_xs, d_w, d_b, nullptr, nullptr, nullptr, workspace, workspace_bytes, stream);
}

static int gru_grads_g4_impl(int count, const int* ns, int d, const float* const* xs, const int32_t* const* x_rows, const float* const* hdecs,
                             const float* const* g4s, const float* const* w_ihs, float* const* d_xs, float* d_w, float* d_b,
                             const uint32_t* const* g4_row_keys, const uint32_t* const* g4_col_keys, const uint32_t* const* x_col_keys,
                             void* workspace, size_t workspace_bytes, void* stream) {
  if (count <= 0 || count > WG_MAXG || !ns || !xs || !hdecs || !g4s || !w_ihs || !d_xs || !d_w || !d_b) return TEMP_E_BADARG;
  WgArgs a = {};
  if (!grads_g4_plan(count, ns, d, &a)) return TEMP_E_UNSUPPORTED;
  for (int i = 0; i < count; ++i) {
    if (!xs[i] || !hdecs[i] || !g4s[i] || !w_ihs[i]) return TEMP_E_UNSUPPORTED;
    a.g[i] = WgGroup{ns[i], g4s[i], xs[i], hdecs[i]};
  }
  const WgWs ws = wg_workspace(a);
  if (!workspace || workspace_bytes < ws.total) return TEMP_E_WORKSPACE;
  char* base = (char*)workspace;
  a.part = (float*)(base + ws.part); a.bpart = (float*)(base + ws.bpart);
  a.part2 = (float*)(base + ws.part2); a.bpart2 = (float*)(base + ws.bpart2);
  hipStream_t st = (hipStream_t)stream;
  int rc;
  bool hx = hx_enabled() && g4_col_keys != nullptr;
  for (int i = 0; i < count && hx; ++i) hx = g4_col_keys[i] != nullptr;
  if (x_rows && (!hx || wgx_rows_lds_bytes(wg_col_tiles(d) < 8 ? wg_col_tiles(d) : 8, a.rows_per_slice) > WGX_LDS_MAX)) return TEMP_E_UNSUPPORTED;
  PanelBatch<EpiStore> batch;
  int nx = 0;
  for (int i = 0; i < count; ++i)
    if (d_xs[i]) batch.p[nx++] = PanelProblem<EpiStore>{ns[i], g4s[i], nullptr, w_ihs[i], EpiStore{d_xs[i], d}, (hx && g4_row_keys) ? g4_row_keys[i] : nullptr};
  for (int i = nx; i < PANEL_MAXP && nx > 0; ++i) { batch.p[i] = batch.p[0]; batch.p[i].M = 0; }
  SideScope side(st);
  const bool beside = nx > 0 && (option(TEMP_OPT_DEBUG) & 0x10000) && side_fork(side);
  if (beside) {
    rc = launch_gemm_panel_multi(K_GEMM_GRU_DX, batch, nx, d, 3 * d, 4 * d, d, 0, side.ss->s);
    if (!side_done(side) || rc) return rc ? rc : TEMP_E_LAUNCH;
  }
  if (hx) {
    WgxKeys keys = {};
    unsigned* xk = (unsigned*)(base + ws.xkeys);
    for (int i = 0; i < count; ++i) {
      keys.g[i] = g4_col_keys[i];
      if (x_col_keys && x_col_keys[i]) { keys.x[i] = x_col_keys[i]; continue; }
      keys.x[i] = xk + (size_t)i * d;
      launch_absmax_keys(ns[i], d, xs[i], d, nullptr, xk + (size_t)i * d, xk + (size_t)count * d + (size_t)i * ABSMAX_BLOCKS * d, st);
    }
    if (x_rows) {
      WgxRows rows = {};
      for (int i = 0; i < count; ++i) rows.r[i] = x_rows[i];
      switch (wg_col_tiles(d)) {
        case 1: rc = launch_gru_wgrad_hx_rows<1>(a, keys, rows, st); break;
        case 2: rc = launch_gru_wgrad_hx_rows<2>(a, keys, rows, st); break;
        case 3: rc = launch_gru_wgrad_hx_rows<3>(a, keys, rows, st); break;
        case 4: rc = launch_gru_wgrad_hx_rows<4>(a, keys, rows, st); break;
        case 5: rc = launch_gru_wgrad_hx_rows<5>(a, keys, rows, st); break;
        case 6: rc = launch_gru_wgrad_hx_rows<6>(a, keys, rows, st); break;
        case 7: rc = launch_gru_wgrad_hx_rows<7>(a, keys, rows, st); break;
        default: rc = launch_gru_wgrad_hx_rows<8>(a, keys, rows, st); break;
      }
    } else
    switch (wg_col_tiles(d)) {
      case 1: rc = launch_gru_wgrad_hx<1>(a, keys, st); break;
      case 2: rc = launch_gru_wgrad_hx<2>(a, keys, st); break;
      case 3: rc = launch_gru_wgrad_hx<3>(a, keys, st); break;
      case 4: rc = launch_gru_wgrad_hx<4>(a, keys, st); break;
      case 5: rc = launch_gru_wgrad_hx<5>(a, keys, st); break;
      case 6: rc = launch_gru_wgrad_hx<6>(a, keys, st); break;
      case 7: rc = launch_gru_wgrad_hx<7>(a, keys, st); break;
      default: rc = launch_gru_wgrad_hx<8>(a, keys, st); break;
    }
  } else
  switch (wg_col_tiles(d)) {
    case 1: rc = launch_gru_wgrad<1>(a, st); break;
    case 2: rc = launch_gru_wgrad<2>(a, st); break;
    case 3: rc = launch_gru_wgrad<3>(a, st); break;
    case 4: rc = launch_gru_wgrad<4>(a, st); break;
    case 5: rc = launch_gru_wgrad<5>(a, st); break;
    case 6: rc = launch_gru_wgrad<6>(a, st); break;
    case 7: rc = launch_gru_wgrad<7>(a, st); break;
    default: rc = launch_gru_wgrad<8>(a, st); break;
  }
  if (rc) return rc;
  const int Ka = 3 * d, R0 = a.tail ? 256 * a.fb : Ka, S2 = a.tail ? a.S * a.P : 0;
  const long long quads = (long long)2 * count * Ka * (d / 4);
  int gx = ceil_div(quads, 256);
  if (gx > 2048) gx = 2048;
  TEMP_LAUNCH(K_REDUCE_SLICES, k_gru_wgrad_reduce, dim3(gx), dim3(256), 0, st, 2 * count, Ka, d, a.S, a.part, a.bpart, R0, S2, a.part2, a.bpart2, d_w, d_b);
  if (beside) {
    const int jr = side.join();
    return jr ? jr : launch_status();
  }
  if (nx > 0) rc = launch_gemm_panel_multi(K_GEMM_GRU_DX, batch, nx, d, 3 * d, 4 * d, d, 0, st);
  return rc ? rc : launch_status();
}

int temp_gru_grads_g4_keys(int count, const int* ns, int d, const float* const* xs, const float* const* hdecs, const float* const* g4s,
                           const float* const* w_ihs, float* const* d_xs, float* d_w, float* d_b, const uint32_t* const* g4_row_keys,
                           const uint32_t* const* g4_col_keys, const uint32_t* const* x_col_keys, void* workspace, size_t workspace_bytes,
                           void* stream) {
  return gru_grads_g4_impl(count, ns, d, xs, nullptr, hdecs, g4s, w_ihs, d_xs, d_w, d_b, g4_row_keys, g4_col_keys, x_col_keys, workspace,
                           workspace_bytes, stream);
}

int temp_gru_grads_g4_rows_supported(int count, const int* ns, int d, int table_rows) {
  WgArgs a = {};
  if (table_rows <= 0 || !hx_enabled() || !grads_g4_plan(count, ns, d, &a)) return 0;
  if ((unsigned long long)table_rows * (unsigned long long)d * 4ull >= (1ull << 32)) return 0;
  for (int i = 0; i < count; ++i)
    if ((unsigned long long)ns[i] * (unsigned long long)d * 4ull >= (1ull << 32)) return 0;
  return wgx_rows_lds_bytes(wg_col_tiles(d) < 8 ? wg_col_tiles(d) : 8, a.rows_per_slice) <= WGX_LDS_MAX ? 1 : 0;
}

int temp_gru_grads_g4_rows(int count, const int* ns, int d, const float* table, int table_rows, const int32_t* const* x_rows,
                           const float* const* hdecs, const float* const* g4s, const float* const* w_ihs, float* const* d_xs, float* d_w,
                           float* d_b, const uint32_t* const* g4_row_keys, const uint32_t* const* g4_col_keys,
                           const uint32_t* const* x_col_keys, void* workspace, size_t workspace_bytes, void* stream) {
  if (count <= 0 || count > WG_MAXG || !table || table_rows <= 0 || !x_rows || !g4_row_keys || !g4_col_keys || !x_col_keys) return TEMP_E_BADARG;
  if (!ns || !temp_gru_grads_g4_rows_supported(count, ns, d, table_rows)) return TEMP_E_UNSUPPORTED;
  const float* xs[WG_MAXG];
  for (int i = 0; i < count; ++i) {
    if (!x_rows[i] || !g4_col_keys[i] || !x_col_keys[i]) return TEMP_E_BADARG;
    xs[i] = table;
  }
  return gru_grads_g4_impl(count, ns, d, xs, x_rows, hdecs, g4s, w_ihs, d_xs, d_w, d_b, g4_row_keys, g4_col_keys, x_col_keys, workspace,
                           workspace_bytes, stream);
}

}
```

### temp_amd/csrc/rgcn_kernels.hip

```cpp
#include <stdlib.h>
#include <atomic>
#include <mutex>
#include "common.hpp"
#include "side_stream.hpp"

namespace temp {

enum { MODE_FWD = 0, MODE_DX = 1 };

template <int S, int MODE>
__device__ __forceinline__ void block_mac(float4& acc, const float4 x, const float4* w, const float c) {
  if (S == 1) {
    acc.x = fmaf(c * x.x, w[0].x, acc.x);
    acc.y = fmaf(c * x.y, w[0].y, acc.y);
    acc.z = fmaf(c * x.z, w[0].z, acc.z);
    acc.w = fmaf(c * x.w, w[0].w, acc.w);
  } else if (S == 2) {
    const float x0 = c * x.x, x1 = c * x.y, x2 = c * x.z, x3 = c * x.w;
    if (MODE == MODE_FWD) {
      acc.x = fmaf(x0, w[0].x, fmaf(x1, w[0].z, acc.x));
      acc.y = fmaf(x0, w[0].y, fmaf(x1, w[0].w, acc.y));
      acc.z = fmaf(x2, w[1].x, fmaf(x3, w[1].z, acc.z));
      acc.w = fmaf(x2, w[1].y, fmaf(x3, w[1].w, acc.w));
    } else {
// ... 411 lines not shown
__host__ __device__ inline int fix_huge(int n_partial) { const int h = (n_partial + FIX_LIST_CAP - 2) / (FIX_LIST_CAP - 1); return h > 2048 ? h : 2048; }
inline int fix_list_cap(int n_partial) { return n_partial / fix_huge(n_partial) + 1; }
inline size_t fix_ctl_bytes(int n_partial, size_t width) { return align_up((size_t)(FIX_LIST + (1 + (width + 255) / 256) * fix_list_cap(n_partial)) * sizeof(unsigned), 256); }
inline size_t fix_scratch_rows(int n_partial) { return (size_t)n_partial / FIX_PART + fix_list_cap(n_partial); }
inline size_t partial_bytes(int n_partial, size_t width) {
  size_t b = align_up((size_t)n_partial * width * sizeof(float), 256);
  if (n_partial >= FIX_SPLIT_MIN) b += fix_ctl_bytes(n_partial, width) + align_up(fix_scratch_rows(n_partial) * width * sizeof(float), 256);
  return b;
}

__global__ void __launch_bounds__(256) k_fixup_split(const int32_t* __restrict__ fix_seg, const int32_t* __restrict__ fix_slot,
                                                     const int32_t* __restrict__ fix_cnt, const float* __restrict__ partial, int width,
                                                     float* __restrict__ out, unsigned* __restrict__ ctl, int cap, float* __restrict__ scratch) {
  __shared__ int pre[FIX_LIST_CAP + 1];
  __shared__ float4 share[4][64];
  __shared__ int last_flag;
  const int n_h = (int)ctl[0];
  if (n_h == 0) return;
  const int tid = threadIdx.x, lane = tid & 63, wave = __builtin_amdgcn_readfirstlane(tid >> 6);
  const int cblocks = (width + 255) >> 8;
  for (int j = tid; j < n_h; j += blockDim.x) pre[j + 1] = (fix_cnt[ctl[FIX_LIST + j]] + FIX_PART - 1) / FIX_PART;
  __syncthreads();
  if (tid == 0) { pre[0] = 0; int run = 0; for (int j = 1; j <= n_h; ++j) { run += pre[j]; pre[j] = run; } }
  __syncthreads();
  const int total = pre[n_h] * cblocks;
  unsigned* ticket = ctl + FIX_LIST + cap;
  for (int w = blockIdx.x; w < total; w += gridDim.x) {
    const int pw = w / cblocks, cb = w - pw * cblocks;
    int lo = 0, hi = n_h;
    while (hi - lo > 1) { const int mid = (lo + hi) >> 1; if (pre[mid] <= pw) lo = mid; else hi = mid; }
    const int j = lo, part = pw - pre[j], parts = pre[j + 1] - pre[j];
    const int i = (int)ctl[FIX_LIST + j];
    const int seg = fix_seg[i], slot0 = fix_slot[i], cnt = fix_cnt[i];
    const int f = (cb << 8) + (lane << 2);
    const int p0 = part * FIX_PART, p1 = min(cnt, p0 + FIX_PART);
    const int per = (p1 - p0 + 3) >> 2;
    const int s0 = min(p1, p0 + wave * per), s1 = min(p1, s0 + per);
    share[wave][lane] = f < width ? fixup_walk(partial + (size_t)slot0 * width + f, s0, s1, width) : zero4();
    __syncthreads();
    if (wave == 0 && f < width)
      st4(scratch + (size_t)(pre[j] + part) * width + f, add4(add4(share[0][lane], share[1][lane]), add4(share[2][lane], share[3][lane])));
    __threadfence();
    __syncthreads();
    if (tid == 0) last_flag = atomicAdd(&ticket[j * cblocks + cb], 1u) == (unsigned)(parts - 1);
    __syncthreads();
    if (last_flag) {
      __threadfence();
      if (wave == 0 && f < width) st4(out + (size_t)seg * width + f, fixup_walk(scratch + (size_t)pre[j] * width + f, 0, parts, width));
    }
    __syncthreads();
  }
}

template <int S>
__global__ void __launch_bounds__(256) k_rgcn_dw(TempEdgeView v, const float* __restrict__ x, const int32_t* __restrict__ x_ids,
                                                 const float* __restrict__ dz, const float* __restrict__ nnorm, int D, int lpr,
                                                 float* __restrict__ dW, float* __restrict__ partial) {
  const int lane = threadIdx.x & 63, wave = threadIdx.x >> 6, wpb = blockDim.x >> 6;
  const int lr = lane & (lpr - 1), gi = lane / lpr, epw = 64 / lpr;
  const int f = lr << 2;
  const bool active = f < D;
  const int wrow = D * S;
  ItemRange it = xcd_chunks(v.n_chunks, v.n_edges, v.chunk_beg, wpb);
  for (int c = it.beg + wave; c < it.end; c += it.stride) {
    const int seg = v.chunk_seg[c], cbeg = v.chunk_beg[c], cend = v.chunk_end[c], slot = v.chunk_slot[c];
    float4 acc[S];
#pragma unroll
    for (int j = 0; j < S; ++j) acc[j] = zero4();
    for (int beg = cbeg; beg < cend; beg += 64) {
      const int cnt = min(64, cend - beg);
      int a_l = 0, b_l = 0;
      float s_l = 0.f;
      if (lane < cnt) {
        a_l = v.a[beg + lane];
        if (x_ids) a_l = x_ids[a_l];
        b_l = v.b[beg + lane];
        const float nn = nnorm[b_l];
        s_l = nn * nn;
      }
      constexpr int U = 4;
      for (int e0 = 0; e0 < cnt; e0 += epw * U) {
        float4 xv[U], gv[U];
        float sc[U];
#pragma unroll
        for (int u = 0; u < U; ++u) {
          const int e = e0 + u * epw + gi;
          const bool ok = (e < cnt) && active;
          const int src = __shfl(a_l, e & 63), dst = __shfl(b_l, e & 63);
          sc[u] = __shfl(s_l, e & 63);
          xv[u] = ok ? ld4(x + (size_t)src * D + f) : zero4();
          gv[u] = ok ? ld4(dz + (size_t)dst * D + f) : zero4();
        }
#pragma unroll
        for (int u = 0; u < U; ++u) {
          const float4 g = scale4(gv[u], sc[u]);
          const float4 xx = xv[u];
          if (S == 1) {
            acc[0].x = fmaf(xx.x, g.x, acc[0].x);
            acc[0].y = fmaf(xx.y, g.y, acc[0].y);
            acc[0].z = fmaf(xx.z, g.z, acc[0].z);
            acc[0].w = fmaf(xx.w, g.w, acc[0].w);
          } else if (S == 2) {
            acc[0].x = fmaf(xx.x, g.x, acc[0].x);
            acc[0].y = fmaf(xx.x, g.y, acc[0].y);
            acc[0].z = fmaf(xx.y, g.x, acc[0].z);
            acc[0].w = fmaf(xx.y, g.y, acc[0].w);
// ... 179 lines not shown
  int S = 0;
  bool fixed = false;
  const int wres = (mode == MODE_FWD) ? d_out : d_in;
  if (fast_shape(d_in, d_out, num_bases, &S)) {
#define TEMP_AGG(SS)                                                                                   \
  if (mode == MODE_FWD) fixed = launch_agg<SS, MODE_FWD>(v, mb, 0, feat, ldf, ids, W, n_rel_rows, nnorm, d_in, out, partial, st); \
  else fixed = launch_agg<SS, MODE_DX>(v, mb, 1, feat, ldf, ids, W, n_rel_rows, nnorm, d_in, out, partial, st);
    if (S == 1) { TEMP_AGG(1) } else if (S == 2) { TEMP_AGG(2) } else { TEMP_AGG(4) }
#undef TEMP_AGG
  } else {
    const int si = d_in / num_bases, so = d_out / num_bases;
    int grid = (v.n_chunks + 3) / 4;
    if (grid > 4096) grid = 4096;
    if (mode == MODE_FWD)
      TEMP_LAUNCH(K_RGCN_AGG_FWD, (k_rgcn_agg_generic<MODE_FWD>), dim3(grid), dim3(256), 0, st, v, feat, ldf, ids, W, nnorm, d_in, d_out, si, so,
                         out, partial);
    else
      TEMP_LAUNCH(K_RGCN_AGG_DX, (k_rgcn_agg_generic<MODE_DX>), dim3(grid), dim3(256), 0, st, v, feat, ldf, ids, W, nnorm, d_in, d_out, si, so,
                         out, partial);
    rgcn_route_count(mode == MODE_FWD ? TEMP_RGCN_FWD_GENERIC : TEMP_RGCN_DX_GENERIC, 0);
  }
  if (!fixed) launch_fixup(v, partial, wres, out, st);
  return launch_status();
}

template <int S>
static bool launch_dw_tile(const TempEdgeView& v, const TileArgs& t, const float* x, const int32_t* x_ids, const float* dz, const float* nnorm, int D,
                           float* dW, float* partial, hipStream_t st) {
  static const bool granted = tile_grant_lds(k_rgcn_dw_t<S>, TILE_LDS_MAX);
  if (!granted) { (void)hipGetLastError(); return false; }
  const int grid = 8 * ceil_div(t.n_members, 8) * t.n_slices;
  TEMP_LAUNCH(K_RGCN_DW, (k_rgcn_dw_t<S>), dim3(grid), dim3(TILE_THREADS), t.lds_bytes, st, v, t, x, x_ids, dz, nnorm, D, dW, partial);
  g_tile_launches.fetch_add(1, std::memory_order_relaxed);
  rgcn_route_count(TEMP_RGCN_DW_TILE, S);
  return true;
}

template <int S>
static bool launch_dw_hybrid(const TempEdgeView& v, const TileArgs& t, const float* x, const int32_t* x_ids, const float* dz, const float* nnorm, int D,
                             float* dW, float* partial, hipStream_t st) {
  static const bool granted = tile_grant_lds(k_rgcn_dw_h<S>, TILE_LDS_MAX);
  if (!granted) { (void)hipGetLastError(); return false; }
  const int grid = 8 * ceil_div(t.n_members, 8) * t.n_slices;
  TEMP_LAUNCH(K_RGCN_DW, (k_rgcn_dw_h<S>), dim3(grid), dim3(TILE_THREADS), t.lds_bytes, st, v, t, x, x_ids, dz, nnorm, D, dW, partial);
  g_tile_launches.fetch_add(1, std::memory_order_relaxed);
  rgcn_route_count(TEMP_RGCN_DW_HYBRID, S);
  return true;
}

static int run_dw(const TempEdgeView& v, const TempMembers* mb, const float* x, const int32_t* x_ids, const float* dz, const float* nnorm, int d_in, int d_out, int num_bases,
                  int n_rel_rows, float* dW, float* partial, hipStream_t st) {
  const int si = d_in / num_bases, so = d_out / num_bases;
  const size_t wrow = (size_t)num_bases * si * so;
  if (hipMemsetAsync(dW, 0, (size_t)n_rel_rows * wrow * sizeof(float), st) != hipSuccess) return TEMP_E_LAUNCH;
  if (v.n_chunks == 0) return TEMP_OK;
  int S = 0;
  TileArgs ta;
  if (fast_shape(d_in, d_out, num_bases, &S) && mb && option(TEMP_OPT_RGCN_TILE) >= 3 && n_rel_rows <= 65535 && v.n_partial < 0xffffff &&
      tile_plan(*mb, 2, d_in, S, 0, 0, 4, &ta) &&
      (S == 1 ? launch_dw_hybrid<1>(v, ta, x, x_ids, dz, nnorm, d_in, dW, partial, st)
              : S == 2 ? launch_dw_hybrid<2>(v, ta, x, x_ids, dz, nnorm, d_in, dW, partial, st) : launch_dw_hybrid<4>(v, ta, x, x_ids, dz, nnorm, d_in, dW, partial, st))) {
  } else if (fast_shape(d_in, d_out, num_bases, &S) && mb && option(TEMP_OPT_RGCN_TILE) == 2 && n_rel_rows <= 65535 && v.n_partial < 0xffffff &&
      tile_plan(*mb, 2, d_in, S, 1, 0, 2, &ta) &&
      (S == 1 ? launch_dw_tile<1>(v, ta, x, x_ids, dz, nnorm, d_in, dW, partial, st)
              : S == 2 ? launch_dw_tile<2>(v, ta, x, x_ids, dz, nnorm, d_in, dW, partial, st) : launch_dw_tile<4>(v, ta, x, x_ids, dz, nnorm, d_in, dW, partial, st))) {
  } else if (fast_shape(d_in, d_out, num_bases, &S)) {
    const int lpr = pick_lpr(d_in);
    int grid = (v.n_chunks + 3) / 4;
    grid = grid < 8 ? 8 : (grid > 2048 ? 2048 : (grid + 7) / 8 * 8);
    if (lpr == 64 && !rgcn_scalar_off()) {
      if (S == 1) TEMP_LAUNCH(K_RGCN_DW, (k_rgcn_dw_s<1>), dim3(grid), dim3(256), 0, st, v, x, x_ids, dz, nnorm, d_in, dW, partial);
      else if (S == 2) TEMP_LAUNCH(K_RGCN_DW, (k_rgcn_dw_s<2>), dim3(grid), dim3(256), 0, st, v, x, x_ids, dz, nnorm, d_in, dW, partial);
      else TEMP_LAUNCH(K_RGCN_DW, (k_rgcn_dw_s<4>), dim3(grid), dim3(256), 0, st, v, x, x_ids, dz, nnorm, d_in, dW, partial);
      rgcn_route_count(TEMP_RGCN_DW_SCALAR, S);
    } else {
      if (S == 1) TEMP_LAUNCH(K_RGCN_DW, (k_rgcn_dw<1>), dim3(grid), dim3(256), 0, st, v, x, x_ids, dz, nnorm, d_in, lpr, dW, partial);
      else if (S == 2) TEMP_LAUNCH(K_RGCN_DW, (k_rgcn_dw<2>), dim3(grid), dim3(256), 0, st, v, x, x_ids, dz, nnorm, d_in, lpr, dW, partial);
      else TEMP_LAUNCH(K_RGCN_DW, (k_rgcn_dw<4>), dim3(grid), dim3(256), 0, st, v, x, x_ids, dz, nnorm, d_in, lpr, dW, partial);
      rgcn_route_count(TEMP_RGCN_DW_PERMUTE, S);
    }
  } else {
    int grid = (v.n_chunks + 3) / 4;
    if (grid > 4096) grid = 4096;
    TEMP_LAUNCH(K_RGCN_DW, k_rgcn_dw_generic, dim3(grid), dim3(256), 0, st, v, x, x_ids, dz, nnorm, d_in, d_out, si, so, dW, partial);
    rgcn_route_count(TEMP_RGCN_DW_GENERIC, 0);
  }
  launch_fixup(v, partial, (int)wrow, dW, st);
  return launch_status();
}

__global__ void __launch_bounds__(256) k_loop_gather_epi(int n, int d4, const int32_t* __restrict__ ids, const int32_t* __restrict__ in_deg,
                                                         const float4* __restrict__ t_loop, const float4* __restrict__ bias, int act,
                                                         DropSpec drop, float4* __restrict__ out) {
  const size_t total = (size_t)n * d4;
  for (size_t i = (size_t)blockIdx.x * blockDim.x + threadIdx.x; i < total; i += (size_t)gridDim.x * blockDim.x) {
    const int row = (int)(i / (unsigned)d4), c = (int)(i - (size_t)row * d4);
    float4 v = in_deg[row] > 0 ? out[i] : zero4();
    float4 lm = t_loop[(size_t)ids[row] * d4 + c];
    if (drop.p > 0.f) lm = drop4(drop, (unsigned)row, (unsigned)c * 4, lm);
    v = add4(v, lm);
    if (bias) v = add4(v, bias[c]);
    if (act == TEMP_ACT_RELU) v = make_float4(fmaxf(v.x, 0.f), fmaxf(v.y, 0.f), fmaxf(v.z, 0.f), fmaxf(v.w, 0.f));
    out[i] = v;
  }
}

template <class Tail>
static int dw_forked(SideScope& sc, const TempEdgeView& v, const TempMembers* mb, const float* x, const int32_t* x_ids, const float* dz,
                     const float* nnorm, int d_in, int d_out, int num_bases, int n_rel_rows, float* dW, float* partial, Tail tail) {
  SideStream* ss = sc.ss;
  if (hipEventRecord(ss->fork, sc.st) != hipSuccess) return TEMP_E_LAUNCH;
  if (hipStreamWaitEvent(ss->s, ss->fork, 0) != hipSuccess) return TEMP_E_LAUNCH;
  sc.forked = true;
  int rc = run_dw(v, mb, x, x_ids, dz, nnorm, d_in, d_out, num_bases, n_rel_rows, dW, partial, ss->s);
  if (!rc) rc = tail(ss->s);
  if (hipEventRecord(ss->join, ss->s) != hipSuccess) return TEMP_E_LAUNCH;
  sc.join_recorded = true;
  return rc;
}
static int dw_forked(SideScope& sc, const TempEdgeView& v, const TempMembers* mb, const float* x, const int32_t* x_ids, const float* dz,
                     const float* nnorm, int d_in, int d_out, int num_bases, int n_rel_rows, float* dW, float* partial) {
  return dw_forked(sc, v, mb, x, x_ids, dz, nnorm, d_in, d_out, num_bases, n_rel_rows, dW, partial, [](hipStream_t) { return (int)TEMP_OK; });
}

static std::atomic<long long> g_pair_launches{0};

template <int S>
__global__ void __launch_bounds__(256) k_pair_msg(int n_rows, int n_table, int D, const float* __restrict__ table, const float* __restrict__ W,
                                                  float* __restrict__ M) {
  const int D4 = D >> 2;
  const size_t total = (size_t)n_rows * D4;
  for (size_t i = (size_t)blockIdx.x * blockDim.x + threadIdx.x; i < total; i += (size_t)gridDim.x * blockDim.x) {
    const int row = (int)(i / (unsigned)D4), f = ((int)(i - (size_t)row * D4)) << 2;
    const int r = row / n_table, e = row - r * n_table;
    const float* wr = W + (size_t)r * (D * S) + f * S;
    float4 w[S];
#pragma unroll
    for (int j = 0; j < S; ++j) w[j] = ld4(wr + 4 * j);
    float4 acc = zero4();
    block_mac<S, MODE_FWD>(acc, ld4(table + (size_t)e * D + f), w, 1.f);
    st4(M + (size_t)row * D + f, acc);
  }
}

template <bool SCALE>
__device__ __forceinline__ float4 pair_rows_sum(const int32_t* __restrict__ idx, int beg, int end, const float* __restrict__ rows, int D,
                                                const float* __restrict__ nnorm, int lane, bool active) {
  float4 acc = zero4();
  const int f = lane << 2;
  for (int b0 = beg; b0 < end; b0 += 64) {
    const int cnt = min(64, end - b0);
    int r_l = 0;
    float s_l = 0.f;
    if (lane < cnt) {
      r_l = idx[b0 + lane];
      if (SCALE) { const float nn = nnorm[r_l]; s_l = nn * nn; }
    }
    if (active) {
      auto row = [&](int i) { return ld4(rows + (size_t)__builtin_amdgcn_readlane(r_l, i) * D + f); };
      auto add = [&](int i, const float4 x) {
        if (SCALE) acc = fma4(__builtin_bit_cast(float, __builtin_amdgcn_readlane(__builtin_bit_cast(int, s_l), i)), x, acc);
        else acc = add4(acc, x);
      };
      int e = 0;
      for (; e + 8 <= cnt; e += 8) {
        float4 x[8];
#pragma unroll
        for (int u = 0; u < 8; ++u) x[u] = row(e + u);
#pragma unroll
        for (int u = 0; u < 8; ++u) add(e + u, x[u]);
      }
      for (; e + 2 <= cnt; e += 2) {
// ... 503 lines not shown
  hipStream_t st = (hipStream_t)stream;
  float* partial = (float*)workspace;
  rc = run_agg(MODE_FWD, g->by_dst, members_of(g), h, d_in, h_ids, weight, n_rel_rows, g->nnorm, d_in, d_out, num_bases, out, partial, st);
  if (rc) return rc;
  const DropSpec ds = drop_spec(drop);
  return gemm_add_bias_act(K_GEMM_LOOP_FWD, g->n_nodes, d_out, d_in, h, d_in, h_ids, loop_w, d_out, 0, out, d_out, g->in_deg, bias, act, out, d_out, st, &ds);
}

struct BwdWs {
  float* dz;
  float* dzm;
  float* part_dx;
  float* part_dw;
  LoopWs loop;
  size_t total;
};
static BwdWs carve_bwd(const TempGraph* g, int d_in, int d_out, int num_bases, char* base) {
  BwdWs w;
  Carver c(base);
  w.dz = (float*)c.take((size_t)g->n_nodes * d_out * sizeof(float));
  w.dzm = (float*)c.take((size_t)g->n_nodes * d_out * sizeof(float));
  w.part_dx = (float*)c.take(partial_bytes(g->by_src.n_partial, d_in));
  w.part_dw = (float*)c.take(partial_bytes(g->by_rel.n_partial, weight_row(d_in, d_out, num_bases)));
  w.loop = carve_loop(c, g->n_nodes, g->n_nodes, d_in, d_out);
  w.total = c.total();
  return w;
}

size_t temp_rgcn_bwd_workspace(const TempGraph* g, int d_in, int d_out, int num_bases, int n_rel_rows) {
  (void)n_rel_rows;
  if (!g || num_bases <= 0 || d_in <= 0 || d_out <= 0) return 0;
  return carve_bwd(g, d_in, d_out, num_bases, nullptr).total;
}

int temp_rgcn_bwd(const TempGraph* g, const float* h, const float* out, const float* d_out_grad, int d_in, int d_out, int num_bases,
                  int n_rel_rows, const float* weight, const float* loop_w, int has_bias, int act, float* d_h, float* d_weight,
                  float* d_loop_w, float* d_bias, void* workspace, size_t workspace_bytes, const TempDropout* drop, void* stream) {
  if (!g || !h || !d_out_grad || !weight || !loop_w || !d_h || !d_weight || !d_loop_w) return TEMP_E_BADARG;
  int rc = layer_shape(d_in, d_out, num_bases, n_rel_rows);
  if (rc) return rc;
  if (grad_args(act, out, has_bias, d_bias)) return TEMP_E_BADARG;
  if (!view_ok(g->by_src) || !rel_view_ok(g, n_rel_rows) || (g->n_nodes > 0 && (!g->nnorm || !g->out_deg))) return TEMP_E_BADARG;
  if (!workspace || workspace_bytes < temp_rgcn_bwd_workspace(g, d_in, d_out, num_bases, n_rel_rows)) return TEMP_E_WORKSPACE;
  hipStream_t st = (hipStream_t)stream;
  if (g->n_nodes == 0) return zero_grads(d_in, d_out, n_rel_rows, weight_row(d_in, d_out, num_bases), has_bias, d_weight, d_loop_w, d_bias, st);
  BwdWs w = carve_bwd(g, d_in, d_out, num_bases, (char*)workspace);
  const float *dz, *dzm;
  rc = grad_dz(act, (size_t)g->n_nodes * d_out, out, d_out_grad, w.dz, st, &dz);
  if (rc) return rc;
  SideScope side(st);
  SideStream* ss = side.ss;
  const DropSpec ds = drop_spec(drop);
  const bool tail_beside = ss && !(ds.p > 0.f) && !(option(TEMP_OPT_DEBUG) & 0x20000);
  if (ss) {
    rc = dw_forked(side, g->by_rel, members_of(g), h, nullptr, dz, g->nnorm, d_in, d_out, num_bases, n_rel_rows, d_weight, w.part_dw,
                   [&](hipStream_t s2) {
                     if (!tail_beside) return (int)TEMP_OK;
                     return loop_grads(w.loop, g->n_nodes, d_in, d_out, h, dz, g->n_nodes, dz, has_bias, d_loop_w, d_bias, s2);
                   });
    if (rc) return rc;
  }
  rc = run_agg(MODE_DX, g->by_src, members_of(g), dz, d_out, nullptr, weight, n_rel_rows, g->nnorm, d_in, d_out, num_bases, d_h, w.part_dx, st);
  if (rc) return rc;
  rc = grad_dzm(ds, g->n_nodes, d_out, dz, w.dzm, st, &dzm);
  if (rc) return rc;
  rc = gemm_add_bias_act(K_GEMM_LOOP_DX, g->n_nodes, d_in, d_out, dzm, d_out, nullptr, loop_w, d_out, 1, d_h, d_in, g->out_deg, nullptr, TEMP_ACT_NONE,
                         d_h, d_in, st);
  if (rc) return rc;
  if (!ss) {
    rc = run_dw(g->by_rel, members_of(g), h, nullptr, dz, g->nnorm, d_in, d_out, num_bases, n_rel_rows, d_weight, w.part_dw, st);
    if (rc) return rc;
  }
  rc = tail_beside ? (int)TEMP_OK : loop_grads(w.loop, g->n_nodes, d_in, d_out, h, dzm, g->n_nodes, dz, has_bias, d_loop_w, d_bias, st);
  return rc ? rc : side.join();
}

int temp_rgcn_bwd_dh(const TempGraph* g, const float* out, const float* d_out_grad, int d_in, int d_out, int num_bases, int n_rel_rows,
                     const float* weight, const float* loop_w, int act, float* d_h, float* dz_out, float* dzm_out, void* workspace,
                     size_t workspace_bytes, const TempDropout* drop, void* stream) {
  if (!g || !d_out_grad || !weight || !loop_w || !d_h) return TEMP_E_BADARG;
  int rc = layer_shape(d_in, d_out, num_bases, n_rel_rows);
  if (rc) return rc;
  if (!act_ok(act) || (act == TEMP_ACT_RELU && (!out || !dz_out))) return TEMP_E_BADARG;
  if (!view_ok(g->by_src) || (g->n_nodes > 0 && (!g->nnorm || !g->out_deg))) return TEMP_E_BADARG;
  if (!workspace || workspace_bytes < temp_rgcn_bwd_workspace(g, d_in, d_out, num_bases, n_rel_rows)) return TEMP_E_WORKSPACE;
  if (g->n_nodes == 0) return TEMP_OK;
  const DropSpec ds = drop_spec(drop);
  if (ds.p > 0.f && !dzm_out) return TEMP_E_BADARG;
  hipStream_t st = (hipStream_t)stream;
  BwdWs w = carve_bwd(g, d_in, d_out, num_bases, (char*)workspace);
  const float *dz, *dzm;
  rc = grad_dz(act, (size_t)g->n_nodes * d_out, out, d_out_grad, dz_out, st, &dz);
  if (rc) return rc;
  rc = run_agg(MODE_DX, g->by_src, members_of(g), dz, d_out, nullptr, weight, n_rel_rows, g->nnorm, d_in, d_out, num_bases, d_h, w.part_dx, st);
  if (rc) return rc;
  rc = grad_dzm(ds, g->n_nodes, d_out, dz, dzm_out, st, &dzm);
  if (rc) return rc;
  return gemm_add_bias_act(K_GEMM_LOOP_DX, g->n_nodes, d_in, d_out, dzm, d_out, nullptr, loop_w, d_out, 1, d_h, d_in, g->out_deg, nullptr, TEMP_ACT_NONE,
                           d_h, d_in, st);
}

int temp_rgcn_bwd_weights(const TempGraph* g, const float* h, const float* dz, const float* dzm, int d_in, int d_out, int num_bases, int n_rel_rows,
                          int has_bias, float* d_weight, float* d_loop_w, float* d_bias, void* workspace, size_t workspace_bytes, void* stream) {
  if (!g || !h || !dz || !d_weight || !d_loop_w) return TEMP_E_BADARG;
  int rc = layer_shape(d_in, d_out, num_bases, n_rel_rows);
  if (rc) return rc;
  if (has_bias && !d_bias) return TEMP_E_BADARG;
  if (!rel_view_ok(g, n_rel_rows) || (g->n_nodes > 0 && !g->nnorm)) return TEMP_E_BADARG;
  if (!workspace || workspace_bytes < temp_rgcn_bwd_workspace(g, d_in, d_out, num_bases, n_rel_rows)) return TEMP_E_WORKSPACE;
  hipStream_t st = (hipStream_t)stream;
  if (g->n_nodes == 0) return zero_grads(d_in, d_out, n_rel_rows, weight_row(d_in, d_out, num_bases), has_bias, d_weight, d_loop_w, d_bias, st);
  BwdWs w = carve_bwd(g, d_in, d_out, num_bases, (char*)workspace);
  rc = run_dw(g->by_rel, members_of(g), h, nullptr, dz, g->nnorm, d_in, d_out, num_bases, n_rel_rows, d_weight, w.part_dw, st);
  if (rc) return rc;
  rc = loop_grads(w.loop, g->n_nodes, d_in, d_out, h, dzm ? dzm : dz, g->n_nodes, dz, has_bias, d_loop_w, d_bias, st);
  return rc ? rc : launch_status();
// ... 47 lines not shown
```

### temp_amd/gru_chain.py

```python
import numpy as np
import torch

from . import _hostlib, _lib
from .backend import get_backend


CHAIN_KERNELS = True
WEIGHT_GRADS_MULTI = True
KEYED_GRADS = True
GATE_GRADS_ONCE = True
FUSED_INPUT_GATES = True
ROWS_IN_PLACE = True


class GruInstance:
    __slots__ = ("n", "x0", "h0", "rnn", "prev", "next", "prev_idx", "next_idx", "dt", "group")

    def __init__(self, n, x0, rnn, prev, prev_idx_np, dt_np, next_idx_np=None):
        self.n, self.x0, self.rnn, self.prev = int(n), int(x0), rnn, prev
        self.h0 = 0
        self.next = -1
        self.prev_idx = prev_idx_np
        self.next_idx = next_idx_np
        self.dt = dt_np
# ... 285 lines not shown
    else:
        packs = be.gru_chain_pack_multi(w_hh) if hasattr(be, "gru_chain_pack_multi") else [be.gru_chain_pack(w) for w in w_hh]
    be.gru_chain_fwd(tabs, gi, lam, variant, packs, b_hh, H, saved, gi_index=gi_index, **decay, **offset)
    return packs


def _position_forward(be, prog, gi, W, lam, variant, H, saved):
    tens = prog.upload(H.device)
    _, none_idx = prog.constants(H.device, H.shape[1])
    for level in prog.levels:
        cells = []
        for i in level:
            it = prog.inst[i]
            p = prog.inst[it.prev] if it.prev >= 0 else None
            cells.append(dict(gi=gi[it.h0:it.h0 + it.n], prev=H[p.h0:p.h0 + p.n] if p is not None else None,
                              prev_idx=tens[i][0] if p is not None else none_idx[:it.n], dt=tens[i][2], w_hh=W[it.rnn][1], b_hh=W[it.rnn][3],
                              h_out=H[it.h0:it.h0 + it.n], row0=it.h0))
        be.gru_cell_fwd_multi(cells, lam, variant, saved)


def _gate_grads_g4(be, ctx, saved, ups, W, decay, offset):
    N, d, dev = saved.shape[1], saved.shape[2], saved.device
    g4 = torch.empty(N, 4 * d, dtype=torch.float32, device=dev)
    keys = None
    if KEYED_GRADS and not offset and hasattr(be, "gru_chain_keys_supported") and be.gru_chain_keys_supported(d):
        keys = (torch.empty(N, dtype=torch.int32, device=dev), torch.empty(ctx.n_rnn + ctx.tabs["n_panels"], 4 * d, dtype=torch.int32, device=dev))
    be.gru_chain_bwd_g4(ctx.tabs, saved, ups, ctx.lam, ctx.variant, ctx.packs, [w[3] for w in W], g4,
                        **({"keys": keys} if keys is not None else {}), **decay, **offset)
    return g4, keys


def _gate_grads_chain(be, ctx, saved, ups, W, decay, offset, dgi, dgh):
    be.gru_chain_bwd(ctx.tabs, saved, ups, ctx.lam, ctx.variant, ctx.packs, [w[3] for w in W], dgi, dgh, **decay, **offset)


def _gate_grads_positions(be, ctx, saved, ups, W, dgi, dgh):
    prog, dev = ctx.prog, saved.device
    tens = prog.upload(dev)
    decv = torch.empty(prog.n_total, dtype=torch.float32, device=dev)
    d_prev = torch.empty(prog.n_total, saved.shape[2], dtype=torch.float32, device=dev)
    given = dict(zip(ctx.want, ups)) if ctx.want is not None else None
    for level in reversed(prog.levels):
        cells = []
        for i in level:
            it = prog.inst[i]
            nxt = prog.inst[it.next] if (it.next >= 0 and prog.inst[it.next].n > 0) else None
            sl = slice(it.h0, it.h0 + it.n)
            cells.append(dict(row0=it.h0, n=it.n, dh_up=ups[0][sl] if given is None else given.get(i),
                              d_prev_next=d_prev[nxt.h0:nxt.h0 + nxt.n] if nxt is not None else None, next_idx=tens[i][1] if nxt is not None else None,
                              dt=tens[i][2], w_hh=W[it.rnn][1], dgi=dgi[sl], dgh=dgh[sl], decv=decv[sl], d_prev=d_prev[sl], no_prev=it.prev < 0))
        be.gru_cell_bwd_multi(cells, ctx.lam, ctx.variant, saved)


def _weight_grads_g4(be, ctx, x_all, saved, g4, keys, W, d_x_all):
    groups, (xsl, hsl) = ctx.prog.groups, _group_rows(ctx.prog.groups)
    kw = dict(row_keys=[keys[0][b] for b in hsl], col_keys=[keys[1][g["rnn"]] for g in groups]) if keys is not None else {}
    if keys is not None and ctx.x_keys is not None:
        kw["x_col_keys"] = [ctx.x_keys[1]] * len(groups)
    return be.gru_grads_g4([x_all[a] for a in xsl], [saved[4, b] for b in hsl], [g4[b] for b in hsl], [W[g["rnn"]][0] for g in groups],
                           [d_x_all[a] for a in xsl], **kw)


def _weight_grads_multi(be, ctx, x_all, saved, dgi, dgh, W, d_x_all):
    xsl, hsl = _group_rows(ctx.prog.groups)
    return be.gru_weight_grads_multi([x_all[a] for a in xsl], [saved[4, b] for b in hsl], [dgi[b] for b in hsl], [dgh[b] for b in hsl],
                                     [W[g["rnn"]][0] for g in ctx.prog.groups], ctx.variant, [d_x_all[a] for a in xsl])


def _weight_grads_per_group(be, ctx, x_all, saved, dgi, dgh, W, zero_state, d_x_all):
    written, out = np.zeros(x_all.shape[0], dtype=bool), []
    for g, zero, xs, hs in zip(ctx.prog.groups, zero_state, *_group_rows(ctx.prog.groups)):
        first = not written[xs].any()
        assert first or written[xs].all()
        tgt = d_x_all[xs] if first else torch.empty_like(d_x_all[xs])
        out.append(be.gru_weight_grads(x_all[xs], None if zero else saved[4, hs], dgi[hs], dgh[hs], W[g["rnn"]][0], ctx.variant, tgt))
        if not first:
            d_x_all[xs] += tgt
        written[xs] = True
    return out


def _scatter_grads(ctx, per_group, d_x_all):
    grads, covered = [None] * (4 * ctx.n_rnn), np.zeros(d_x_all.shape[0], dtype=bool)
    for g, gw in zip(ctx.prog.groups, per_group):
        covered[g["x0"]:g["x1"]] = True
        for k in range(4):
            j = 4 * g["rnn"] + k
            grads[j] = gw[k] if grads[j] is None else grads[j] + gw[k]
    if not covered.all():
        d_x_all[torch.from_numpy(~covered).to(d_x_all.device)] = 0
    return grads


def _backward_result(be, ctx, d_x_all, grads, decay, offset):
    d_dec, d_off = (None, None), (None, None, None)
    if decay:
        d_wb = be.gru_chain_decay_reduce(ctx.tabs, d_x_all.shape[1], ctx.variant, decay["d_arg"], ctx.n_rnn)
        d_dec = (d_wb[:, 0].sum().reshape(1, 1), d_wb[:, 1].sum().reshape(1))
    if offset:
        seg_ptr, order = ctx.off_inverse
        d_off = (be.segment_sum_rows(offset["d_state"], seg_ptr, order, ctx.off_rows), None, None)
    return (d_x_all, None, None, None, None, None, None) + d_dec + d_off + tuple(grads)


def _grads_strategy(be, prog, d, variant, on_chain):
    groups = prog.groups
    zero_state = [all(it.prev < 0 for it in prog.inst if it.group == gi) for gi in range(len(groups))]
    disjoint = all(groups[a]["x1"] <= groups[b]["x0"] or groups[b]["x1"] <= groups[a]["x0"] for a in range(len(groups)) for b in range(a))
    one_launch = bool(groups and disjoint and not any(zero_state) and len({g["rnn"] for g in groups}) == len(groups) and WEIGHT_GRADS_MULTI)
    once = one_launch and GATE_GRADS_ONCE and on_chain and be.gru_grads_g4_supported([g["h1"] - g["h0"] for g in groups], d, variant)
    return zero_state, one_launch, once

# ... 56 lines not shown
            d_x_all = torch.empty_like(x_all)
            per_group = _weight_grads_g4(be, ctx, x_all, saved, g4, keys, W, d_x_all)
        else:
            dgi, dgh = new(N, ctx.G), new(N, 3 * d)
            if ctx.tabs is not None:
                _gate_grads_chain(be, ctx, saved, ups, W, decay, offset, dgi, dgh)
            else:
                _gate_grads_positions(be, ctx, saved, ups, W, dgi, dgh)
            d_x_all = torch.empty_like(x_all)
            per_group = _weight_grads_multi(be, ctx, x_all, saved, dgi, dgh, W, d_x_all) if one_launch else None
            if per_group is None:
                per_group = _weight_grads_per_group(be, ctx, x_all, saved, dgi, dgh, W, zero_state, d_x_all)
        return _backward_result(be, ctx, d_x_all, _scatter_grads(ctx, per_group, d_x_all), decay, offset)


class _GruChainRowsFn(torch.autograd.Function):

    @staticmethod
    def forward(ctx, table, prog, inverse, relu_table, lam, variant, n_rnn, want, *weights):
        be = get_backend()
        dev, d, N = table.device, table.shape[1], prog.n_total
        table = table.detach().contiguous()
        W = [tuple(w.detach().contiguous() for w in weights[4 * r:4 * r + 4]) for r in range(n_rnn)]
        tabs, x_rows = prog.chain_tables(dev, want), prog.x_rows(dev)
        x_col_keys = be.absmax_keys(table, rows=False)[1]
        H, saved = torch.empty(N, d, dtype=torch.float32, device=dev), torch.empty(5, N, d, dtype=torch.float32, device=dev)
        w_ih, w_hh, b_ih, b_hh = ([w[k] for w in W] for k in range(4))
        packs = be.gru_chain_pack_x_multi(w_hh, w_ih)
        be.gru_chain_fwd_x(tabs, table, x_rows, lam, variant, packs, b_hh, b_ih, H, saved)
        ctx.set_materialize_grads(False)
        ctx.save_for_backward(table, saved, x_rows, x_col_keys, *[w for ws in W for w in ws])
        ctx.prog, ctx.lam, ctx.variant, ctx.n_rnn, ctx.want, ctx.tabs, ctx.packs = prog, lam, variant, n_rnn, want, tabs, packs
        ctx.inverse, ctx.relu_table = inverse, relu_table
        if want is None:
            return H
        return tuple(H[prog.inst[i].h0:prog.inst[i].h0 + prog.inst[i].n] for i in want)

    @staticmethod
    def backward(ctx, *d_outs):
        be = get_backend()
        table, saved, x_rows, x_col_keys = ctx.saved_tensors[:4]
        W = [ctx.saved_tensors[4 + 4 * r:8 + 4 * r] for r in range(ctx.n_rnn)]
        prog, groups = ctx.prog, ctx.prog.groups
        d, N = table.shape[1], prog.n_total
        if ctx.want is None:
            ups = [d_outs[0].contiguous() if d_outs[0] is not None else torch.zeros(N, d, dtype=torch.float32, device=table.device)]
        else:
            given = {i: g.contiguous() for i, g in zip(ctx.want, d_outs) if g is not None}
            ups = [given.get(i) for i in ctx.want]
        g4, keys = _gate_grads_g4(be, ctx, saved, ups, W, {}, {})
        xsl, hsl = _group_rows(groups)
        d_x_all = torch.empty(prog.x_rows_count, d, dtype=torch.float32, device=table.device)
        per_group = be.gru_grads_g4_rows(table, [x_rows[b] for b in hsl], [saved[4, b] for b in hsl], [g4[b] for b in hsl],
                                         [W[g["rnn"]][0] for g in groups], [d_x_all[a] for a in xsl], row_keys=[keys[0][b] for b in hsl],
                                         col_keys=[keys[1][g["rnn"]] for g in groups], x_col_keys=[x_col_keys] * len(groups))
        grads = _scatter_grads(ctx, per_group, d_x_all)
        seg_ptr, order = ctx.inverse
        d_table = be.segment_sum_rows(d_x_all, seg_ptr, order, table.shape[0], relu_of=table if ctx.relu_table else None)
        return (d_table, None, None, None, None, None, None, None) + tuple(grads)


def rows_in_place_usable(prog, table, inverse, n_rnn, type1=False, want=None, decay=None, offset=None):
    be = get_backend()
    dev, d = table.device, table.shape[1]
    variant = _lib.GRU_TYPE1 if type1 else _lib.GRU_TORCH
    if not (ROWS_IN_PLACE and hasattr(be, "gru_grads_g4_rows") and decay is None and offset is None and variant == _lib.GRU_TORCH):
        return False
    if inverse is None or d % 4 or d > 256 or table.shape[0] * d * 4 >= 2 ** 32 or prog.x_rows(dev) is None or prog.x_rows_max > table.shape[0]:
        return False
    tabs = prog.chain_tables(dev, tuple(want) if want is not None else None) if chain_kernels_usable(d, n_rnn) else None
    if tabs is None or not (FUSED_INPUT_GATES and hasattr(be, "gru_chain_fwd_x") and be.gru_chain_fwd_x_supported(d, variant, tabs["max_steps"])):
        return False
    if not (KEYED_GRADS and hasattr(be, "gru_chain_keys_supported") and be.gru_chain_keys_supported(d) and be.keys_supported(d)):
        return False
    return bool(_grads_strategy(be, prog, d, variant, True)[2]
                and be.gru_grads_g4_rows_supported([g["h1"] - g["h0"] for g in prog.groups], d, variant, table.shape[0]))


def chain_kernels_usable(d, n_rnn=1):
    be = get_backend()
    return bool(CHAIN_KERNELS and n_rnn <= _lib.CHAIN_MAX_RNN and be.gru_chain_supported(d))


def chain_decay_usable(d, variant, n_rnn=1):
    be = get_backend()
    return bool(chain_kernels_usable(d, n_rnn) and hasattr(be, "gru_chain_decay_supported") and be.gru_chain_decay_supported(d, variant))


def chain_offset_usable(d, variant, n_rnn=1):
    be = get_backend()
    return bool(chain_kernels_usable(d, n_rnn) and hasattr(be, "gru_chain_offset_supported") and be.gru_chain_offset_supported(d, variant))


def offset_tables(index_np, n_rows, device):
    from .functional import gather_inverse
    index_np = np.asarray(index_np).reshape(-1)
    return _lib.to_device(index_np.astype(np.int32), device), gather_inverse(index_np, int(n_rows), device)


def program_on_chain_kernels(prog, device, want):
    return prog.chain_tables(device, tuple(want) if want is not None else None) is not None


def prepare_program(prog, device, d, n_rnn, want, chain_rows=None):
    if chain_kernels_usable(d, n_rnn) and prog.chain_tables(device, tuple(want) if want is not None else None) is not None:
        _lib.pause_point()
        prog.gi_shared(device)
# ... 38 lines not shown
```

Before: 968.3 million.

## Prepack w_ih for backward dx GEMM and replace dW memset with empty-row zeroing

Adds a new chain pack layout (HX_XD) that also stores a pre-packed w_ih operand for the backward dx GEMM. The g4 gradient kernels can then reuse it instead of repacking w_ih on every backward call. Separately, the RGCN dW full memset is replaced by a single-block kernel that zeroes only relation rows with no chunks, run after accumulation. A debug-gated option to run the aggregation before forking the dW side stream is also added. The trade-offs are a larger pack buffer and a serial one-block zeroing kernel on the stream.

```diff
diff --git a/include/temp_amd.h b/include/temp_amd.h
--- a/include/temp_amd.h
+++ b/include/temp_amd.h
@@ -259,12 +259,14 @@
 int temp_gru_grads_g4_keys(int count, const int* ns, int d, const float* const* xs, const float* const* hdecs, const float* const* g4s,
                            const float* const* w_ihs, float* const* d_xs, float* d_w, float* d_b, const uint32_t* const* g4_row_keys,
                            const uint32_t* const* g4_col_keys, const uint32_t* const* x_col_keys ,
-                           void* workspace, size_t workspace_bytes, void* stream);
+                           const float* const* packed ,
+                           int pack_layout, void* workspace, size_t workspace_bytes, void* stream);
 int temp_gru_grads_g4_rows_supported(int count, const int* ns, int d, int table_rows);
 int temp_gru_grads_g4_rows(int count, const int* ns, int d, const float* table, int table_rows, const int32_t* const* x_rows,
                            const float* const* hdecs, const float* const* g4s, const float* const* w_ihs, float* const* d_xs, float* d_w,
                            float* d_b, const uint32_t* const* g4_row_keys, const uint32_t* const* g4_col_keys,
-                           const uint32_t* const* x_col_keys, void* workspace, size_t workspace_bytes, void* stream);
+                           const uint32_t* const* x_col_keys, const float* const* packed, int pack_layout, void* workspace,
+                           size_t workspace_bytes, void* stream);
 
 #define TEMP_CHAIN_HAS_PREV (1 << 30)
 #define TEMP_CHAIN_TRACKS 32
@@ -287,7 +289,7 @@
   const TempChainDecay* decay;
   const TempChainOffset* offset;
 } TempGruChain;
-enum { TEMP_CHAIN_PACK_F32 = 1, TEMP_CHAIN_PACK_BX = 2, TEMP_CHAIN_PACK_HX = 3, TEMP_CHAIN_PACK_HX_X = 4 };
+enum { TEMP_CHAIN_PACK_F32 = 1, TEMP_CHAIN_PACK_BX = 2, TEMP_CHAIN_PACK_HX = 3, TEMP_CHAIN_PACK_HX_X = 4, TEMP_CHAIN_PACK_HX_XD = 5 };
 int temp_gru_chain_pack_layout(int d);
 int temp_gru_chain_supported(int d);
 size_t temp_gru_chain_pack_floats(int d);
@@ -295,7 +297,10 @@
 int temp_gru_chain_pack_multi(int count, int d, const float* const* w_hh, float* const* packed, void* stream);
 int temp_gru_chain_pack_multi_layout(int layout, int count, int d, const float* const* w_hh, float* const* packed, void* stream);
 size_t temp_gru_chain_pack_x_floats(int d);
+size_t temp_gru_chain_pack_dx_offset(int d);
 int temp_gru_chain_pack_x_multi(int count, int d, const float* const* w_hh, const float* const* w_ih, float* const* packed, void* stream);
+int temp_gru_chain_pack_x_multi_layout(int layout, int count, int d, const float* const* w_hh, const float* const* w_ih, float* const* packed,
+                                       void* stream);
 typedef struct TempChainFwd {
   const float* gi; const float* x; const int32_t* x_index; const float* const* b_ih;
   float* h_out; float* saved;
diff --git a/temp_amd/_lib.py b/temp_amd/_lib.py
--- a/temp_amd/_lib.py
+++ b/temp_amd/_lib.py
@@ -56,7 +56,7 @@
 CHAIN_MAX_RNN = 4
 CHAIN_MAX_UP = 8
 CHAIN_MAX_STEPS = 64
-CHAIN_PACK_F32, CHAIN_PACK_BX, CHAIN_PACK_HX, CHAIN_PACK_HX_X = 1, 2, 3, 4
+CHAIN_PACK_F32, CHAIN_PACK_BX, CHAIN_PACK_HX, CHAIN_PACK_HX_X, CHAIN_PACK_HX_XD = 1, 2, 3, 4, 5
 
 
 class TempChainDecay(ctypes.Structure):
@@ -181,7 +181,9 @@
     "temp_gru_chain_pack_layout": (_I, [_I]),
     "temp_gru_chain_fwd_x_supported": (_I, [_I, _I, _I]),
     "temp_gru_chain_pack_x_floats": (_SZ, [_I]),
+    "temp_gru_chain_pack_dx_offset": (_SZ, [_I]),
     "temp_gru_chain_pack_x_multi": (_I, [_I, _I, ctypes.POINTER(c_vp), ctypes.POINTER(c_vp), ctypes.POINTER(c_vp), c_vp]),
+    "temp_gru_chain_pack_x_multi_layout": (_I, [_I, _I, _I, ctypes.POINTER(c_vp), ctypes.POINTER(c_vp), ctypes.POINTER(c_vp), c_vp]),
     "temp_gru_chain_fwd_x_launches": (ctypes.c_longlong, []),
     "temp_gru_chain_bwd": (_I, [ctypes.POINTER(TempGruChain), ctypes.POINTER(TempChainBwd), c_vp]),
     "temp_gru_chain_keys_supported": (_I, [_I]),
@@ -193,9 +195,9 @@
     "temp_gru_chain_offset_layout": (_I, [_I]),
     "temp_gru_chain_pack_multi_layout": (_I, [_I, _I, _I, ctypes.POINTER(c_vp), ctypes.POINTER(c_vp), c_vp]),
     "temp_gru_chain_offset_launches": (ctypes.c_longlong, []),
-    "temp_gru_grads_g4_keys": (_I, [_I, c_vp, _I, c_vp, c_vp, c_vp, c_vp, c_vp, c_vp, c_vp, c_vp, c_vp, c_vp, c_vp, ctypes.c_size_t, c_vp]),
+    "temp_gru_grads_g4_keys": (_I, [_I, c_vp, _I, c_vp, c_vp, c_vp, c_vp, c_vp, c_vp, c_vp, c_vp, c_vp, c_vp, c_vp, _I, c_vp, ctypes.c_size_t, c_vp]),
     "temp_gru_grads_g4_rows_supported": (_I, [_I, c_vp, _I, _I]),
-    "temp_gru_grads_g4_rows": (_I, [_I, c_vp, _I, c_vp, _I, c_vp, c_vp, c_vp, c_vp, c_vp, c_vp, c_vp, c_vp, c_vp, c_vp, c_vp, ctypes.c_size_t, c_vp]),
+    "temp_gru_grads_g4_rows": (_I, [_I, c_vp, _I, c_vp, _I, c_vp, c_vp, c_vp, c_vp, c_vp, c_vp, c_vp, c_vp, c_vp, c_vp, c_vp, _I, c_vp, ctypes.c_size_t, c_vp]),
     "temp_gru_grads_g4_workspace": (ctypes.c_size_t, [_I, c_vp, _I]),
     "temp_gru_grads_g4": (_I, [_I, c_vp, _I, c_vp, c_vp, c_vp, c_vp, c_vp, c_vp, c_vp, c_vp, ctypes.c_size_t, c_vp]),
     "temp_gather_rows": (_I, [_I, _I, c_vp, c_vp, c_vp, c_vp]),
diff --git a/temp_amd/backend.py b/temp_amd/backend.py
--- a/temp_amd/backend.py
+++ b/temp_amd/backend.py
@@ -490,16 +490,29 @@
     def gru_chain_fwd_x_supported(self, d, variant, max_steps):
         return bool(self.lib.temp_gru_chain_fwd_x_supported(int(d), int(variant), int(max_steps)))
 
-    def gru_chain_pack_x_multi(self, w_hhs, w_ihs):
+    def gru_chain_pack_x_multi(self, w_hhs, w_ihs, layout=None):
         w_hhs, w_ihs = [_f32(w, "w_hh") for w in w_hhs], [_f32(w, "w_ih") for w in w_ihs]
         d = w_hhs[0].shape[1]
         k = len(w_hhs)
         n = self.lib.temp_gru_chain_pack_x_floats(d)
         buf = torch.empty(k, n, dtype=torch.float32, device=w_hhs[0].device)
         arr = lambda ts: (ctypes.c_void_p * k)(*[t.data_ptr() for t in ts])
+        if layout is not None:
+            _lib.check(self.lib.temp_gru_chain_pack_x_multi_layout(int(layout), k, d, arr(w_hhs), arr(w_ihs), arr([buf[i] for i in range(k)]), _stream()),
+                       "temp_gru_chain_pack_x_multi_layout")
+            return self._tagged([buf[i] for i in range(k)], int(layout))
         _lib.check(self.lib.temp_gru_chain_pack_x_multi(k, d, arr(w_hhs), arr(w_ihs), arr([buf[i] for i in range(k)]), _stream()),
                    "temp_gru_chain_pack_x_multi")
-        return self._tagged([buf[i] for i in range(k)], _lib.CHAIN_PACK_HX_X)
+        return self._tagged([buf[i] for i in range(k)], _lib.CHAIN_PACK_HX_XD)
+
+    @staticmethod
+    def _w_ih_packs(w_ihs):
+        if not any(isinstance(w, (tuple, list)) for w in w_ihs):
+            return list(w_ihs), None, 0, []
+        packs = [_f32(w[1], "packed") for w in w_ihs]
+        layouts = {getattr(w[1], "chain_pack_layout", None) for w in w_ihs}
+        assert len(layouts) == 1 and None not in layouts, "chain packs without one common layout tag (gru_chain_pack*)"
+        return [w[0] for w in w_ihs], (ctypes.c_void_p * len(packs))(*[p.data_ptr() for p in packs]), int(layouts.pop()), packs
 
     def gru_chain_fwd_x(self, tabs, x, x_index, lam, variant, packs, b_hhs, b_ihs, h_out, saved_all, decay=None):
         d = saved_all.shape[2]
@@ -545,6 +558,7 @@
         return self.lib.temp_gru_grads_g4_workspace(k, (ctypes.c_int * k)(*[int(n) for n in ns]), int(d)) > 0
 
     def gru_grads_g4(self, xs, hdecs, g4s, w_ihs, d_xs, row_keys=None, col_keys=None, x_col_keys=None):
+        w_ihs, pk, pk_layout, pk_keep = self._w_ih_packs(w_ihs)
         k = len(xs)
         d = xs[0].shape[1]
         dev = xs[0].device
@@ -570,7 +584,7 @@
                     assert t.dtype == torch.int32 and t.is_contiguous() and t.numel() == d
                 xk = arr(x_col_keys)
             rc = self.lib.temp_gru_grads_g4_keys(k, ns, d, arr(keep[0]), arr(keep[1]), arr(g4s), arr(keep[2]), dx, _ptr(d_w), _ptr(d_b),
-                                                 arr(row_keys), arr(col_keys), xk, _ptr(ws), ws.numel(), _stream())
+                                                 arr(row_keys), arr(col_keys), xk, pk, pk_layout, _ptr(ws), ws.numel(), _stream())
             _lib.check(rc, "temp_gru_grads_g4_keys")
             return [(d_w[2 * i], d_w[2 * i + 1], d_b[2 * i], d_b[2 * i + 1]) for i in range(k)]
         rc = self.lib.temp_gru_grads_g4(k, ns, d, arr(keep[0]), arr(keep[1]), arr(g4s), arr(keep[2]), dx, _ptr(d_w), _ptr(d_b), _ptr(ws),
@@ -585,6 +599,7 @@
         return bool(self.lib.temp_gru_grads_g4_rows_supported(k, (ctypes.c_int * k)(*[int(n) for n in ns]), int(d), int(table_rows)))
 
     def gru_grads_g4_rows(self, table, x_rows, hdecs, g4s, w_ihs, d_xs, row_keys, col_keys, x_col_keys):
+        w_ihs, pk, pk_layout, pk_keep = self._w_ih_packs(w_ihs)
         table = _f32(table, "table")
         k, d, dev = len(x_rows), table.shape[1], table.device
         ns = (ctypes.c_int * k)(*[r.shape[0] for r in x_rows])
@@ -603,7 +618,8 @@
         d_b = torch.empty(2 * k, 3 * d, dtype=torch.float32, device=dev)
         ws = self._ws(nb, dev)
         rc = self.lib.temp_gru_grads_g4_rows(k, ns, d, _ptr(table), table.shape[0], arr(x_rows), arr(keep[0]), arr(g4s), arr(keep[1]), dx,
-                                             _ptr(d_w), _ptr(d_b), arr(row_keys), arr(col_keys), arr(x_col_keys), _ptr(ws), ws.numel(), _stream())
+                                             _ptr(d_w), _ptr(d_b), arr(row_keys), arr(col_keys), arr(x_col_keys), pk, pk_layout, _ptr(ws), ws.numel(),
+                                             _stream())
         _lib.check(rc, "temp_gru_grads_g4_rows")
         return [(d_w[2 * i], d_w[2 * i + 1], d_b[2 * i], d_b[2 * i + 1]) for i in range(k)]
 
diff --git a/temp_amd/csrc/gemm_bx.hpp b/temp_amd/csrc/gemm_bx.hpp
--- a/temp_amd/csrc/gemm_bx.hpp
+++ b/temp_amd/csrc/gemm_bx.hpp
@@ -604,11 +604,11 @@
 }
 
 template <class Epi>
-int launch_gemm_bx(int kid, const PanelBatch<Epi>& batch, int count, const BxGeom& g, int G, hipStream_t st) {
+int launch_gemm_bx(int kid, const PanelBatch<Epi>& batch, int count, const BxGeom& g, int G, hipStream_t st, const HxPacked* hx_pre = nullptr) {
   if (launch_hxr(kid, batch, count, g, st)) return launch_status();
   if (launch_bxr(kid, batch, count, g, st, nullptr)) return launch_status();
   if (hx_supported(batch, count, g)) {
-    const int rc = launch_gemm_hx(kid, batch, count, g, G, st);
+    const int rc = launch_gemm_hx(kid, batch, count, g, G, st, hx_pre);
     if (rc != TEMP_E_UNSUPPORTED) return rc;
   }
   BxPacked pk;
diff --git a/temp_amd/csrc/gemm_hx.hpp b/temp_amd/csrc/gemm_hx.hpp
--- a/temp_amd/csrc/gemm_hx.hpp
+++ b/temp_amd/csrc/gemm_hx.hpp
@@ -289,7 +289,7 @@
 }
 
 template <class Epi>
-int launch_gemm_hx(int kid, const PanelBatch<Epi>& batch_in, int count, const BxGeom& g, int G, hipStream_t st) {
+int launch_gemm_hx(int kid, const PanelBatch<Epi>& batch_in, int count, const BxGeom& g, int G, hipStream_t st, const HxPacked* pre = nullptr) {
   const size_t pbytes = align_up(hx_pack_bytes(g.N, g.K), 256);
   int n_distinct = 0, which[PANEL_MAXP];
   for (int i = 0; i < count; ++i) {
@@ -305,14 +305,15 @@
   HxPacked pk;
   HxPackJobs jobs = {};
   const size_t items = hx_packed_items(g.N, g.K);
-  int done = 0;
+  bool done[PANEL_MAXP] = {};
   for (int i = 0; i < PANEL_MAXP; ++i) { pk.b[i] = reinterpret_cast<const hx_u32x4*>(slot); pk.keys[i] = reinterpret_cast<const unsigned*>(slot + items * 16); }
   for (int i = 0; i < count; ++i) {
+    if (pre && pre->b[i] && pre->keys[i]) { pk.b[i] = pre->b[i]; pk.keys[i] = pre->keys[i]; continue; }
     unsigned char* dst = slot + (size_t)which[i] * pbytes;
     pk.b[i] = reinterpret_cast<const hx_u32x4*>(dst);
     pk.keys[i] = reinterpret_cast<const unsigned*>(dst + items * 16);
-    if (which[i] < done) continue;
-    ++done;
+    if (done[which[i]]) continue;
+    done[which[i]] = true;
     hx_pack_jobs_add(jobs, batch.p[i].B, reinterpret_cast<hx_u32x4*>(dst), reinterpret_cast<unsigned*>(dst + items * 16), g.K, g.N, g.ldb, g.trans_b);
   }
   int kbo = 0;
diff --git a/temp_amd/csrc/gemm_wres.hpp b/temp_amd/csrc/gemm_wres.hpp
--- a/temp_amd/csrc/gemm_wres.hpp
+++ b/temp_amd/csrc/gemm_wres.hpp
@@ -291,7 +291,8 @@
 inline bool wres_disabled() { return option(TEMP_OPT_GEMM_STREAM) != 0; }
 
 template <class Epi>
-int launch_gemm_panel_multi(int kid, const PanelBatch<Epi>& batch, int count, int N, int K, int lda, int ldb, int trans_b, hipStream_t st) {
+int launch_gemm_panel_multi(int kid, const PanelBatch<Epi>& batch, int count, int N, int K, int lda, int ldb, int trans_b, hipStream_t st,
+                            const HxPacked* hx_pre = nullptr) {
   if (count <= 0 || count > PANEL_MAXP) return TEMP_E_BADARG;
   long long rows = 0;
   for (int i = 0; i < count; ++i) rows += batch.p[i].M > 0 ? batch.p[i].M : 0;
@@ -302,7 +303,7 @@
       for (int i = 0; i < count; ++i) max_m = batch.p[i].M > max_m ? batch.p[i].M : max_m;
       BxGeom bg;
       int G;
-      if (bx_plan(N, K, lda, ldb, trans_b, max_m, rows, &bg, &G)) return launch_gemm_bx(kid, batch, count, bg, G, st);
+      if (bx_plan(N, K, lda, ldb, trans_b, max_m, rows, &bg, &G)) return launch_gemm_bx(kid, batch, count, bg, G, st, hx_pre);
       if (K % 8 == 4 && bx_plan(N, K, lda, ldb, trans_b, max_m, rows, &bg, &G, true) && hx_supported(batch, count, bg)) {
         const int rc = launch_gemm_hx(kid, batch, count, bg, G, st);
         if (rc != TEMP_E_UNSUPPORTED) return rc;
diff --git a/temp_amd/csrc/gru_chain.hip b/temp_amd/csrc/gru_chain.hip
--- a/temp_amd/csrc/gru_chain.hip
+++ b/temp_amd/csrc/gru_chain.hip
@@ -691,9 +691,10 @@
 static bool chain_layout_ok(int layout, int d) {
   if (layout == TEMP_CHAIN_PACK_F32) return true;
   if (layout == TEMP_CHAIN_PACK_BX) return d % 8 == 0;
-  return (layout == TEMP_CHAIN_PACK_HX || layout == TEMP_CHAIN_PACK_HX_X) && chain_hx_fits(d);
-}
-static bool layout_hx(int layout) { return layout == TEMP_CHAIN_PACK_HX || layout == TEMP_CHAIN_PACK_HX_X; }
+  return (layout == TEMP_CHAIN_PACK_HX || layout == TEMP_CHAIN_PACK_HX_X || layout == TEMP_CHAIN_PACK_HX_XD) && chain_hx_fits(d);
+}
+static bool layout_hx(int layout) { return layout == TEMP_CHAIN_PACK_HX || layout == TEMP_CHAIN_PACK_HX_X || layout == TEMP_CHAIN_PACK_HX_XD; }
+static bool layout_x(int layout) { return layout == TEMP_CHAIN_PACK_HX_X || layout == TEMP_CHAIN_PACK_HX_XD; }
 
 static ChainArgs chain_args(const TempGruChain* c, float* d_arg = nullptr, float* d_state = nullptr) {
   ChainArgs a = {};
@@ -997,7 +998,7 @@
 }
 
 static int chain_fwd_x(const TempGruChain* c, const TempChainFwd* io, hipStream_t st) {
-  if (c->pack_layout != TEMP_CHAIN_PACK_HX_X) return TEMP_E_BADARG;
+  if (!layout_x(c->pack_layout)) return TEMP_E_BADARG;
   if (c->variant != TEMP_GRU_TORCH || !chain_fwd_x_fits(c->d, c->max_steps)) return TEMP_E_UNSUPPORTED;
   if (c->n_panels == 0) return TEMP_OK;
   if (!io->x_index || !io->b_ih || !io->h_out || !io->saved) return TEMP_E_BADARG;
@@ -1090,28 +1091,43 @@
   return d > 0 && d % 8 == 0 && variant == TEMP_GRU_TORCH && chain_fwd_x_ok(d, max_steps) ? 1 : 0;
 }
 
+size_t temp_gru_chain_pack_dx_offset(int d) {
+  if (d <= 0) return 0;
+  return chain_x_ih_offset(d) + chain_hx_fwd_items(d) * 4;
+}
+
 size_t temp_gru_chain_pack_x_floats(int d) {
   if (d <= 0) return 0;
-  return chain_x_ih_offset(d) + chain_hx_fwd_items(d) * 4;
-}
-
-int temp_gru_chain_pack_x_multi(int count, int d, const float* const* w_hh, const float* const* w_ih, float* const* packed, void* stream) {
-  if (count <= 0 || count > TEMP_CHAIN_MAX_RNN || d <= 0 || !w_hh || !w_ih || !packed) return TEMP_E_BADARG;
+  return temp_gru_chain_pack_dx_offset(d) + hx_pack_bytes(d, 3 * d) / 4;
+}
+
+int temp_gru_chain_pack_x_multi_layout(int layout, int count, int d, const float* const* w_hh, const float* const* w_ih, float* const* packed,
+                                       void* stream) {
+  if (count <= 0 || count > TEMP_CHAIN_MAX_RNN || d <= 0 || !w_hh || !w_ih || !packed || !layout_x(layout)) return TEMP_E_BADARG;
   for (int i = 0; i < count; ++i) if (!w_hh[i] || !w_ih[i] || !packed[i]) return TEMP_E_BADARG;
   if (d % 8 || !chain_hx(d)) return TEMP_E_UNSUPPORTED;
   const ChainGeomHx gx = chain_geom_hx(d);
+  const int per_gru = layout == TEMP_CHAIN_PACK_HX_XD ? 3 : 2;
   HxPackJobs jobs = {};
   for (int i = 0; i < count; ++i) {
     hx_u32x4* pf = reinterpret_cast<hx_u32x4*>(packed[i]);
     hx_u32x4* pb = pf + chain_hx_fwd_items(d);
     unsigned* kf = reinterpret_cast<unsigned*>(pb + chain_hx_bwd_items(d));
     hx_u32x4* pi = reinterpret_cast<hx_u32x4*>(packed[i] + chain_x_ih_offset(d));
-    if (jobs.count + 2 > HX_PACK_JOBS) { hx_pack_launch(jobs, K_GRU_CHAIN_PACK, (hipStream_t)stream); jobs = HxPackJobs{}; }
+    if (jobs.count + per_gru > HX_PACK_JOBS) { hx_pack_launch(jobs, K_GRU_CHAIN_PACK, (hipStream_t)stream); jobs = HxPackJobs{}; }
     hx_pack_jobs_add_joint(jobs, w_hh[i], pf, w_ih[i], pi, kf, d, 3 * d, d, 1);
     hx_pack_jobs_add(jobs, w_hh[i], pb, kf + gx.NT * 32, 3 * d, d, d, 0, gx.NSb);
+    if (layout == TEMP_CHAIN_PACK_HX_XD) {
+      hx_u32x4* px = reinterpret_cast<hx_u32x4*>(packed[i] + temp_gru_chain_pack_dx_offset(d));
+      hx_pack_jobs_add(jobs, w_ih[i], px, reinterpret_cast<unsigned*>(px + hx_packed_items(d, 3 * d)), 3 * d, d, d, 0);
+    }
   }
   hx_pack_launch(jobs, K_GRU_CHAIN_PACK, (hipStream_t)stream);
   return launch_status();
+}
+
+int temp_gru_chain_pack_x_multi(int count, int d, const float* const* w_hh, const float* const* w_ih, float* const* packed, void* stream) {
+  return temp_gru_chain_pack_x_multi_layout(TEMP_CHAIN_PACK_HX_XD, count, d, w_hh, w_ih, packed, stream);
 }
 
 size_t temp_gru_chain_decay_reduce_workspace(const TempGruChain* c) {
diff --git a/temp_amd/csrc/gru_kernels.hip b/temp_amd/csrc/gru_kernels.hip
--- a/temp_amd/csrc/gru_kernels.hip
+++ b/temp_amd/csrc/gru_kernels.hip
@@ -871,13 +871,14 @@
 int temp_gru_grads_g4(int count, const int* ns, int d, const float* const* xs, const float* const* hdecs, const float* const* g4s,
                       const float* const* w_ihs, float* const* d_xs, float* d_w, float* d_b, void* workspace, size_t workspace_bytes,
                       void* stream) {
-  return temp_gru_grads_g4_keys(count, ns, d, xs, hdecs, g4s, w_ihs, d_xs, d_w, d_b, nullptr, nullptr, nullptr, workspace, workspace_bytes, stream);
+  return temp_gru_grads_g4_keys(count, ns, d, xs, hdecs, g4s, w_ihs, d_xs, d_w, d_b, nullptr, nullptr, nullptr, nullptr, 0, workspace, workspace_bytes,
+                                stream);
 }
 
 static int gru_grads_g4_impl(int count, const int* ns, int d, const float* const* xs, const int32_t* const* x_rows, const float* const* hdecs,
                              const float* const* g4s, const float* const* w_ihs, float* const* d_xs, float* d_w, float* d_b,
                              const uint32_t* const* g4_row_keys, const uint32_t* const* g4_col_keys, const uint32_t* const* x_col_keys,
-                             void* workspace, size_t workspace_bytes, void* stream) {
+                             const float* const* packed, int pack_layout, void* workspace, size_t workspace_bytes, void* stream) {
   if (count <= 0 || count > WG_MAXG || !ns || !xs || !hdecs || !g4s || !w_ihs || !d_xs || !d_w || !d_b) return TEMP_E_BADARG;
   WgArgs a = {};
   if (!grads_g4_plan(count, ns, d, &a)) return TEMP_E_UNSUPPORTED;
@@ -896,14 +897,23 @@
   for (int i = 0; i < count && hx; ++i) hx = g4_col_keys[i] != nullptr;
   if (x_rows && (!hx || wgx_rows_lds_bytes(wg_col_tiles(d) < 8 ? wg_col_tiles(d) : 8, a.rows_per_slice) > WGX_LDS_MAX)) return TEMP_E_UNSUPPORTED;
   PanelBatch<EpiStore> batch;
+  HxPacked dx_pre = {};
+  const bool prepacked = hx && packed && pack_layout == TEMP_CHAIN_PACK_HX_XD;
   int nx = 0;
-  for (int i = 0; i < count; ++i)
-    if (d_xs[i]) batch.p[nx++] = PanelProblem<EpiStore>{ns[i], g4s[i], nullptr, w_ihs[i], EpiStore{d_xs[i], d}, (hx && g4_row_keys) ? g4_row_keys[i] : nullptr};
+  for (int i = 0; i < count; ++i) {
+    if (!d_xs[i]) continue;
+    if (prepacked && packed[i]) {
+      const unsigned char* planes = reinterpret_cast<const unsigned char*>(packed[i] + temp_gru_chain_pack_dx_offset(d));
+      dx_pre.b[nx] = reinterpret_cast<const hx_u32x4*>(planes);
+      dx_pre.keys[nx] = reinterpret_cast<const unsigned*>(planes + hx_packed_items(d, 3 * d) * 16);
+    }
+    batch.p[nx++] = PanelProblem<EpiStore>{ns[i], g4s[i], nullptr, w_ihs[i], EpiStore{d_xs[i], d}, (hx && g4_row_keys) ? g4_row_keys[i] : nullptr};
+  }
   for (int i = nx; i < PANEL_MAXP && nx > 0; ++i) { batch.p[i] = batch.p[0]; batch.p[i].M = 0; }
   SideScope side(st);
   const bool beside = nx > 0 && (option(TEMP_OPT_DEBUG) & 0x10000) && side_fork(side);
   if (beside) {
-    rc = launch_gemm_panel_multi(K_GEMM_GRU_DX, batch, nx, d, 3 * d, 4 * d, d, 0, side.ss->s);
+    rc = launch_gemm_panel_multi(K_GEMM_GRU_DX, batch, nx, d, 3 * d, 4 * d, d, 0, side.ss->s, &dx_pre);
     if (!side_done(side) || rc) return rc ? rc : TEMP_E_LAUNCH;
   }
   if (hx) {
@@ -960,16 +970,16 @@
     const int jr = side.join();
     return jr ? jr : launch_status();
   }
-  if (nx > 0) rc = launch_gemm_panel_multi(K_GEMM_GRU_DX, batch, nx, d, 3 * d, 4 * d, d, 0, st);
+  if (nx > 0) rc = launch_gemm_panel_multi(K_GEMM_GRU_DX, batch, nx, d, 3 * d, 4 * d, d, 0, st, &dx_pre);
   return rc ? rc : launch_status();
 }
 
 int temp_gru_grads_g4_keys(int count, const int* ns, int d, const float* const* xs, const float* const* hdecs, const float* const* g4s,
                            const float* const* w_ihs, float* const* d_xs, float* d_w, float* d_b, const uint32_t* const* g4_row_keys,
-                           const uint32_t* const* g4_col_keys, const uint32_t* const* x_col_keys, void* workspace, size_t workspace_bytes,
-                           void* stream) {
-  return gru_grads_g4_impl(count, ns, d, xs, nullptr, hdecs, g4s, w_ihs, d_xs, d_w, d_b, g4_row_keys, g4_col_keys, x_col_keys, workspace,
-                           workspace_bytes, stream);
+                           const uint32_t* const* g4_col_keys, const uint32_t* const* x_col_keys, const float* const* packed, int pack_layout,
+                           void* workspace, size_t workspace_bytes, void* stream) {
+  return gru_grads_g4_impl(count, ns, d, xs, nullptr, hdecs, g4s, w_ihs, d_xs, d_w, d_b, g4_row_keys, g4_col_keys, x_col_keys, packed, pack_layout,
+                           workspace, workspace_bytes, stream);
 }
 
 int temp_gru_grads_g4_rows_supported(int count, const int* ns, int d, int table_rows) {
@@ -984,7 +994,8 @@
 int temp_gru_grads_g4_rows(int count, const int* ns, int d, const float* table, int table_rows, const int32_t* const* x_rows,
                            const float* const* hdecs, const float* const* g4s, const float* const* w_ihs, float* const* d_xs, float* d_w,
                            float* d_b, const uint32_t* const* g4_row_keys, const uint32_t* const* g4_col_keys,
-                           const uint32_t* const* x_col_keys, void* workspace, size_t workspace_bytes, void* stream) {
+                           const uint32_t* const* x_col_keys, const float* const* packed, int pack_layout, void* workspace,
+                           size_t workspace_bytes, void* stream) {
   if (count <= 0 || count > WG_MAXG || !table || table_rows <= 0 || !x_rows || !g4_row_keys || !g4_col_keys || !x_col_keys) return TEMP_E_BADARG;
   if (!ns || !temp_gru_grads_g4_rows_supported(count, ns, d, table_rows)) return TEMP_E_UNSUPPORTED;
   const float* xs[WG_MAXG];
@@ -992,8 +1003,8 @@
     if (!x_rows[i] || !g4_col_keys[i] || !x_col_keys[i]) return TEMP_E_BADARG;
     xs[i] = table;
   }
-  return gru_grads_g4_impl(count, ns, d, xs, x_rows, hdecs, g4s, w_ihs, d_xs, d_w, d_b, g4_row_keys, g4_col_keys, x_col_keys, workspace,
-                           workspace_bytes, stream);
-}
-
-}
+  return gru_grads_g4_impl(count, ns, d, xs, x_rows, hdecs, g4s, w_ihs, d_xs, d_w, d_b, g4_row_keys, g4_col_keys, x_col_keys, packed, pack_layout,
+                           workspace, workspace_bytes, stream);
+}
+
+}
diff --git a/temp_amd/csrc/rgcn_kernels.hip b/temp_amd/csrc/rgcn_kernels.hip
--- a/temp_amd/csrc/rgcn_kernels.hip
+++ b/temp_amd/csrc/rgcn_kernels.hip
@@ -487,6 +487,29 @@
   }
 }
 
+constexpr int DW_ZERO_MAX_ROWS = 1 << 16, DW_ZERO_MAX_CHUNKS = 1 << 16;
+__global__ void __launch_bounds__(1024) k_dw_zero_empty(int n_rows, int n_chunks, const int32_t* __restrict__ chunk_seg, int wrow, float* __restrict__ dW) {
+  __shared__ unsigned has[DW_ZERO_MAX_ROWS / 32];
+  const int words = (n_rows + 31) >> 5;
+  for (int i = threadIdx.x; i < words; i += 1024) has[i] = 0u;
+  __syncthreads();
+  for (int c0 = threadIdx.x; c0 < n_chunks; c0 += 8 * 1024) {
+    int s[8];
+#pragma unroll
+    for (int u = 0; u < 8; ++u) { const int c = c0 + u * 1024; s[u] = c < n_chunks ? chunk_seg[c] : -1; }
+#pragma unroll
+    for (int u = 0; u < 8; ++u)
+      if ((unsigned)s[u] < (unsigned)n_rows) atomicOr(&has[s[u] >> 5], 1u << (s[u] & 31));
+  }
+  __syncthreads();
+  const int lane = threadIdx.x & 63, wave = __builtin_amdgcn_readfirstlane(threadIdx.x >> 6);
+  for (int r = wave; r < n_rows; r += 16) {
+    if ((has[r >> 5] >> (r & 31)) & 1u) continue;
+    float* row = dW + (size_t)r * wrow;
+    for (int f = lane; f < wrow; f += 64) row[f] = 0.f;
+  }
+}
+
 template <int S>
 __global__ void __launch_bounds__(256) k_rgcn_dw(TempEdgeView v, const float* __restrict__ x, const int32_t* __restrict__ x_ids,
                                                  const float* __restrict__ dz, const float* __restrict__ nnorm, int D, int lpr,
@@ -772,7 +795,9 @@
                   int n_rel_rows, float* dW, float* partial, hipStream_t st) {
   const int si = d_in / num_bases, so = d_out / num_bases;
   const size_t wrow = (size_t)num_bases * si * so;
-  if (hipMemsetAsync(dW, 0, (size_t)n_rel_rows * wrow * sizeof(float), st) != hipSuccess) return TEMP_E_LAUNCH;
+  const bool zero_behind = v.n_chunks > 0 && v.n_chunks <= DW_ZERO_MAX_CHUNKS && n_rel_rows <= DW_ZERO_MAX_ROWS && wrow <= 0x7fffffff &&
+                           option(TEMP_OPT_DEBUG) != 102;
+  if (!zero_behind && hipMemsetAsync(dW, 0, (size_t)n_rel_rows * wrow * sizeof(float), st) != hipSuccess) return TEMP_E_LAUNCH;
   if (v.n_chunks == 0) return TEMP_OK;
   int S = 0;
   TileArgs ta;
@@ -806,6 +831,7 @@
     rgcn_route_count(TEMP_RGCN_DW_GENERIC, 0);
   }
   launch_fixup(v, partial, (int)wrow, dW, st);
+  if (zero_behind) TEMP_LAUNCH(K_RGCN_DW, k_dw_zero_empty, dim3(1), dim3(1024), 0, st, n_rel_rows, v.n_chunks, v.chunk_seg, (int)wrow, dW);
   return launch_status();
 }
 
@@ -827,9 +853,10 @@
 
 template <class Tail>
 static int dw_forked(SideScope& sc, const TempEdgeView& v, const TempMembers* mb, const float* x, const int32_t* x_ids, const float* dz,
-                     const float* nnorm, int d_in, int d_out, int num_bases, int n_rel_rows, float* dW, float* partial, Tail tail) {
+                     const float* nnorm, int d_in, int d_out, int num_bases, int n_rel_rows, float* dW, float* partial, Tail tail,
+                     bool fork_recorded = false) {
   SideStream* ss = sc.ss;
-  if (hipEventRecord(ss->fork, sc.st) != hipSuccess) return TEMP_E_LAUNCH;
+  if (!fork_recorded && hipEventRecord(ss->fork, sc.st) != hipSuccess) return TEMP_E_LAUNCH;
   if (hipStreamWaitEvent(ss->s, ss->fork, 0) != hipSuccess) return TEMP_E_LAUNCH;
   sc.forked = true;
   int rc = run_dw(v, mb, x, x_ids, dz, nnorm, d_in, d_out, num_bases, n_rel_rows, dW, partial, ss->s);
@@ -838,6 +865,7 @@
   sc.join_recorded = true;
   return rc;
 }
+static int dw_fork_point(SideScope& sc) { return hipEventRecord(sc.ss->fork, sc.st) == hipSuccess ? (int)TEMP_OK : (int)TEMP_E_LAUNCH; }
 static int dw_forked(SideScope& sc, const TempEdgeView& v, const TempMembers* mb, const float* x, const int32_t* x_ids, const float* dz,
                      const float* nnorm, int d_in, int d_out, int num_bases, int n_rel_rows, float* dW, float* partial) {
   return dw_forked(sc, v, mb, x, x_ids, dz, nnorm, d_in, d_out, num_bases, n_rel_rows, dW, partial, [](hipStream_t) { return (int)TEMP_OK; });
@@ -1447,16 +1475,24 @@
   SideStream* ss = side.ss;
   const DropSpec ds = drop_spec(drop);
   const bool tail_beside = ss && !(ds.p > 0.f) && !(option(TEMP_OPT_DEBUG) & 0x20000);
+  const bool agg_first = ss && option(TEMP_OPT_DEBUG) == 103;
+  auto side_branch = [&]() {
+    return dw_forked(side, g->by_rel, members_of(g), h, nullptr, dz, g->nnorm, d_in, d_out, num_bases, n_rel_rows, d_weight, w.part_dw,
+                     [&](hipStream_t s2) {
+                       if (!tail_beside) return (int)TEMP_OK;
+                       return loop_grads(w.loop, g->n_nodes, d_in, d_out, h, dz, g->n_nodes, dz, has_bias, d_loop_w, d_bias, s2);
+                     }, agg_first);
+  };
   if (ss) {
-    rc = dw_forked(side, g->by_rel, members_of(g), h, nullptr, dz, g->nnorm, d_in, d_out, num_bases, n_rel_rows, d_weight, w.part_dw,
-                   [&](hipStream_t s2) {
-                     if (!tail_beside) return (int)TEMP_OK;
-                     return loop_grads(w.loop, g->n_nodes, d_in, d_out, h, dz, g->n_nodes, dz, has_bias, d_loop_w, d_bias, s2);
-                   });
+    rc = agg_first ? dw_fork_point(side) : side_branch();
     if (rc) return rc;
   }
   rc = run_agg(MODE_DX, g->by_src, members_of(g), dz, d_out, nullptr, weight, n_rel_rows, g->nnorm, d_in, d_out, num_bases, d_h, w.part_dx, st);
   if (rc) return rc;
+  if (agg_first) {
+    rc = side_branch();
+    if (rc) return rc;
+  }
   rc = grad_dzm(ds, g->n_nodes, d_out, dz, w.dzm, st, &dzm);
   if (rc) return rc;
   rc = gemm_add_bias_act(K_GEMM_LOOP_DX, g->n_nodes, d_in, d_out, dzm, d_out, nullptr, loop_w, d_out, 1, d_h, d_in, g->out_deg, nullptr, TEMP_ACT_NONE,
diff --git a/temp_amd/gru_chain.py b/temp_amd/gru_chain.py
--- a/temp_amd/gru_chain.py
+++ b/temp_amd/gru_chain.py
@@ -361,12 +361,19 @@
         be.gru_cell_bwd_multi(cells, ctx.lam, ctx.variant, saved)
 
 
+def _w_ih_operands(ctx, W, keyed):
+    groups, packs = ctx.prog.groups, ctx.packs
+    if keyed and packs is not None and all(getattr(pk, "chain_pack_layout", None) == _lib.CHAIN_PACK_HX_XD for pk in packs):
+        return [(W[g["rnn"]][0], packs[g["rnn"]]) for g in groups]
+    return [W[g["rnn"]][0] for g in groups]
+
+
 def _weight_grads_g4(be, ctx, x_all, saved, g4, keys, W, d_x_all):
     groups, (xsl, hsl) = ctx.prog.groups, _group_rows(ctx.prog.groups)
     kw = dict(row_keys=[keys[0][b] for b in hsl], col_keys=[keys[1][g["rnn"]] for g in groups]) if keys is not None else {}
     if keys is not None and ctx.x_keys is not None:
         kw["x_col_keys"] = [ctx.x_keys[1]] * len(groups)
-    return be.gru_grads_g4([x_all[a] for a in xsl], [saved[4, b] for b in hsl], [g4[b] for b in hsl], [W[g["rnn"]][0] for g in groups],
+    return be.gru_grads_g4([x_all[a] for a in xsl], [saved[4, b] for b in hsl], [g4[b] for b in hsl], _w_ih_operands(ctx, W, keys is not None),
                            [d_x_all[a] for a in xsl], **kw)
 
 
@@ -529,7 +536,7 @@
         xsl, hsl = _group_rows(groups)
         d_x_all = torch.empty(prog.x_rows_count, d, dtype=torch.float32, device=table.device)
         per_group = be.gru_grads_g4_rows(table, [x_rows[b] for b in hsl], [saved[4, b] for b in hsl], [g4[b] for b in hsl],
-                                         [W[g["rnn"]][0] for g in groups], [d_x_all[a] for a in xsl], row_keys=[keys[0][b] for b in hsl],
+                                         _w_ih_operands(ctx, W, True), [d_x_all[a] for a in xsl], row_keys=[keys[0][b] for b in hsl],
                                          col_keys=[keys[1][g["rnn"]] for g in groups], x_col_keys=[x_col_keys] * len(groups))
         grads = _scatter_grads(ctx, per_group, d_x_all)
         seg_ptr, order = ctx.inverse
```

New measurement: 976.7 million, median of 6. About the same (+0.9%).
